# LBM-EPFL/MaD

Measured on NVIDIA B200. Metric: voxels/sec scale-space+detect+describe(+match), higher is better.
Workload: dtype f32 grids, f64 line accumulation, u8 x u8 -> s32 matching

## Files before the change

### include/mad_b200.h

```cpp
#ifndef MAD_B200_H
#define MAD_B200_H

#include <stddef.h>
#include <stdint.h>

#ifdef __cplusplus
extern "C" {
#endif

#define MAD_OK 0
#define MAD_ERR_ARG (-1)
#define MAD_ERR_CUDA (-2)
#define MAD_ERR_CAPACITY (-3)
#define MAD_ERR_NODEVICE (-4)

#define MAD_MAX_ORI 36
#define MAD_DSC_LEN 1024
#define MAD_DSC_REFUSED (1 << 30)

typedef struct MadKeypoint {
    int32_t vox[3];
    int32_t oct;
    float off[3];
    float val;
    int32_t peak[3];
    int32_t accepted;
} MadKeypoint;

typedef struct MadOriented {
    int32_t kp;
    int16_t main_bin;
    int16_t sec_bin;
} MadOriented;

typedef struct MadZoneTable {
    int32_t n_zones;
    int32_t n_belts;
    const double* bounds;
    const int32_t* belt_first;
    const double* belt_phi;
    const void* fast;
} MadZoneTable;

#define MAD_ZONE_FAST_BYTES 2048
int mad_zone_fast_build(const MadZoneTable* zones_host, void* fast_out, void* stream);

const char* mad_last_error_string(void);
int mad_version(void);
int mad_device_info(int* sm_count, int* cc_major, int* cc_minor);

int mad_publish_small(const void* src_dev, void* dst_host_mapped, int bytes, void* stream);

int mad_copy_to_host(const void* src_dev, void* dst_host_mapped, long long bytes, int n_ctas, void* stream);

long long mad_launch_count(void);
int mad_profile_enable(int on);
int mad_profile_count(void);
int mad_profile_get(int i, const char** name, float* ms);
int mad_profile_reset(void);

int mad_grid_max(const float* grid, long long n, float* out_max_ord, void* stream);
float mad_grid_max_decode(unsigned int ord);
int mad_threshold_normalise(float* grid, long long n, float isovalue, float vmax, int divide, void* stream);
int mad_grid_bbox(const float* grid, int nx, int ny, int nz, int* bbox6, void* stream);
int mad_crop_pad3d(const float* in, int nx, int ny, int nz, int x0, int y0, int z0, int cx, int cy, int cz,
                   int pad, float* out, void* stream);

int mad_pad3d(const float* in, int nx, int ny, int nz, int pad, float* out, void* stream);

size_t mad_upsample_workspace_bytes(int bx, int by, int bz);
int mad_upsample_presmooth(const float* base, int bx, int by, int bz,
                           const double* gauss_w_host, int radius,
                           float* up, void* workspace, size_t workspace_bytes, void* stream);

size_t mad_log_gauss_workspace_bytes(int nx, int ny, int nz);
int mad_log_gauss(const float* grid, int nx, int ny, int nz,
                  const double* w0_host, const double* w2_host, int radius, float scale,
                  float* log_out, float* gauss_out, void* workspace, size_t workspace_bytes,
                  int exact_f64, void* stream);

int mad_gradient(const float* gauss, int nx, int ny, int nz, float* grad4, void* stream);
size_t mad_gradient_tiles(int nx, int ny, int nz);
int mad_gradient_mark(const MadKeypoint* kp, int n_kp, const int* dims_oct_host, int reach_oct0, int reach_oct1,
                      uint8_t* flags_oct0, uint8_t* flags_oct1, void* stream);
int mad_gradient_masked(const float* gauss, int nx, int ny, int nz, float* grad4, uint8_t* flags, void* stream);

int mad_detect(const float* log_grid, int nx, int ny, int nz, int oct, int border,
               float threshold, MadKeypoint* cand, int cap, int* count, void* stream);

size_t mad_sort_keypoints_workspace_bytes(int n);
int mad_sort_keypoints(const MadKeypoint* cand, int n, const int* dims_oct_host,
                       MadKeypoint* out, int* out_count,
                       void* workspace, size_t workspace_bytes, void* stream);

int mad_orient(const float* grad4_oct0, const float* grad4_oct1, const int* dims_oct_host,
               const MadKeypoint* kp, int n_kp, int r, const MadZoneTable* zones112_host,
               const double* r1_table, int lim_main, int lim_sec,
               int32_t* n_ori, int32_t* slots, void* stream);

size_t mad_compact_oriented_workspace_bytes(int n_kp);
int mad_compact_oriented(const int32_t* n_ori, const int32_t* slots, int n_kp,
                         MadOriented* oriented, int cap, int* out_count,
                         void* workspace, size_t workspace_bytes, void* stream);

int mad_describe(const float* grad4_oct0, const float* grad4_oct1, const int* dims_oct_host,
                 const MadKeypoint* kp, const MadOriented* oriented, int n_oriented, int r,
                 const MadZoneTable* zones16_host, const double* rf_table, const double* rf_inv_table,
                 int rf_zones, int16_t* dsc, void* stream);

typedef struct MadDscSet {
    const int16_t* dsc;
    const void* half;
    const int32_t* norm2;
    const uint8_t* u8;
    const float* rnorm;
    int32_t rows;
    int32_t rows_padded;
    int32_t max_entry;
    int32_t max_norm2;
} MadDscSet;

int mad_dsc_prepare(const int16_t* dsc, int rows, int rows_padded, int32_t* norm2, float* rnorm,
                    uint8_t* u8, int32_t* max_entry, int32_t* max_norm2, void* stream);
int mad_dsc_norms(const int16_t* dsc, int rows, int32_t* norm2, void* stream);
int mad_dsc_to_half(const int16_t* dsc, int rows, int rows_padded, void* half_out, void* stream);

int mad_match_segments(int M, int N, int impl);
int mad_match_count(const MadDscSet* hi, const MadDscSet* lo, double cc, int n_seg, int32_t* seg_count, int impl,
                    void* stream);
int mad_match_fill(const MadDscSet* hi, const MadDscSet* lo, double cc, int n_seg, const int64_t* seg_offset,
                   int32_t* pair_hi, int32_t* pair_lo, double* pair_score, int impl, void* stream);
size_t mad_exclusive_scan_workspace_bytes(int n);
int mad_exclusive_scan_i32_to_i64(const int32_t* in, int n, int64_t* out, int64_t* total,
                                  void* workspace, size_t workspace_bytes, void* stream);

int mad_match_pairs(const MadDscSet* hi, const MadDscSet* lo, double cc, uint64_t* cand_key, int32_t* cand_dot,
                    uint64_t cap, uint64_t* count, void* stream);
size_t mad_match_pairs_finish_workspace_bytes(long long n);
int mad_match_pairs_finish(const uint64_t* cand_key, const int32_t* cand_dot, long long n, int hi_rows, int lo_rows,
                           const int32_t* hi_n2, const int32_t* lo_n2, int32_t* pair_hi, int32_t* pair_lo,
                           double* pair_score, void* workspace, size_t workspace_bytes, void* stream);
int mad_match_pairs_finish_dot(const uint64_t* cand_key, const int32_t* cand_dot, long long n, int hi_rows, int lo_rows,
                               int32_t* pair_hi, int32_t* pair_lo, int32_t* pair_dot, void* workspace, size_t workspace_bytes,
                               void* stream);

size_t mad_match_topk_workspace_bytes(int M, int N, int k, int impl);
int mad_match_topk(const MadDscSet* hi, const MadDscSet* lo, int k, int lo_index_base,
                   int32_t* topk_idx, double* topk_score, void* workspace, size_t workspace_bytes,
                   int impl, void* stream);
#define MAD_TOPK_INCOMPLETE (-2)
int mad_topk_merge(const int32_t* idx_in, const double* score_in, int G, int M, int k,
                   int32_t* idx_out, double* score_out, void* stream);

int mad_mark_used(const int32_t* idx, long long n, uint8_t* used, void* stream);
int mad_repeatability(const int32_t* pair_hi, const int32_t* pair_lo, const double* pair_score, long long n_pairs,
                      const double* hi_subv, const double* lo_subv, const int32_t* hi_meta, const int32_t* lo_meta,
                      const double* rf_table, const double* rf_inv_table, int rf_zones,
                      const double* hi_cloud, int n_hi_cloud, const double* lo_sorted, const int32_t* cell_start,
                      const uint32_t* near_bits, const double* grid_org_host, const int* grid_dims_host,
                      double dist, double* results, void* stream);
int mad_repeat_counts(const int32_t* pair_hi, const int32_t* pair_lo, long long p0, long long p1,
                      const double* hi_subv, const double* lo_subv, const int32_t* hi_meta, const int32_t* lo_meta,
                      const double* rf_table, const double* rf_inv_table, int rf_zones,
                      const double* hi_cloud, int n_hi_cloud, const double* lo_sorted, const int32_t* cell_start,
                      const uint32_t* near_bits, const double* grid_org_host, const int* grid_dims_host,
                      double dist, int32_t* counts, void* stream);
int mad_repeat_rows(const int32_t* pair_hi, const int32_t* pair_lo, const double* pair_score, long long n_pairs,
                    const double* hi_subv, const double* lo_subv, const int32_t* hi_meta, const int32_t* lo_meta,
                    const double* rf_table, const double* rf_inv_table, int rf_zones, const int32_t* counts,
                    int n_hi_cloud, double* results, void* stream);

size_t mad_anchor_cloud_workspace_bytes(int n_rows);
int mad_anchor_cloud(const double* subv, const uint8_t* used, int n_rows, double cell, double* cloud, double* grid_org,
                     long long* info, void* workspace, size_t workspace_bytes, void* stream);
size_t mad_cloud_grid_workspace_bytes(int n);
int mad_cloud_grid(const double* cloud, int n, const double* grid_org, const long long* grid_dims_host, double cell,
                   double* sorted, int32_t* cell_start, uint32_t* near_bits, void* workspace, size_t workspace_bytes,
                   void* stream);

int mad_density_splat(const double* xyz, const double* mass, int n_atoms, const double* min_host, double voxelsp,
                      int margin, int px, int py, int pz, double* grid, void* stream);
int mad_normalise_f64(double* grid, long long n, void* scratch8, void* stream);
int mad_conv_full_f64(const double* in, long long outer, int n, long long inner, const double* w_dev, int radius,
                      void* out, int out_is_f32, void* stream);

size_t mad_box_scores_workspace_bytes(int ex, int ey, int ez);
int mad_box_scores(const float* g1, int nx1, int ny1, int nz1, const float* g2, int nx2, int ny2, int nz2,
                   const int* box_host, float isovalue, double* out8, void* workspace, size_t workspace_bytes,
                   void* stream);
int mad_grid_count_gt(const float* grid, long long n, float thr, unsigned long long* out, void* stream);
int mad_mask_with(float* g1, int nx1, int ny1, int nz1, const float* g2, int nx2, int ny2, int nz2,
                  const int* shift_host, const int* lo_host, const int* hi_host, void* stream);
int mad_refine_rigid(const float* grad4, int nx, int ny, int nz, const double* px, const double* py, const double* pz,
                     double voxsp, const double* init, const double* center, const double* max_dist, int n_problems,
                     int n_atoms, int n_steps, double max_step, double min_step, double* coords_out, double* meta_out,
                     void* stream);

#ifdef __cplusplus
}
#endif
#endif
```

### mad_b200/_lib.py

```python
import ctypes as C
import os

import numpy as np

HERE = os.path.dirname(os.path.abspath(__file__))
LIB_PATH = os.path.join(HERE, "libmad_b200.so")


class MadError(RuntimeError):
    pass


if not os.path.exists(LIB_PATH):
    raise ImportError(
        "mad_b200: %s is missing -- build the CUDA library first (python -m mad_b200.build). "
        "There is no CPU fallback." % LIB_PATH)

lib = C.CDLL(LIB_PATH)

KEYPOINT_DTYPE = np.dtype([("vox", "<i4", 3), ("oct", "<i4"), ("off", "<f4", 3), ("val", "<f4"),
                           ("peak", "<i4", 3), ("accepted", "<i4")])
ORIENTED_DTYPE = np.dtype([("kp", "<i4"), ("main", "<i2"), ("sec", "<i2")])
assert KEYPOINT_DTYPE.itemsize == 48 and ORIENTED_DTYPE.itemsize == 8
MAX_ORI = 36
DSC_LEN = 1024
DSC_REFUSED = 1 << 30
TOPK_INCOMPLETE = -2
TOPK_MAX = 32
ZONE_FAST_BYTES = 2048


class MadZoneTable(C.Structure):
    _fields_ = [("n_zones", C.c_int32), ("n_belts", C.c_int32), ("bounds", C.c_void_p),
                ("belt_first", C.c_void_p), ("belt_phi", C.c_void_p), ("fast", C.c_void_p)]


class MadDscSet(C.Structure):
    _fields_ = [("dsc", C.c_void_p), ("half", C.c_void_p), ("norm2", C.c_void_p), ("u8", C.c_void_p),
                ("rnorm", C.c_void_p), ("rows", C.c_int32), ("rows_padded", C.c_int32), ("max_entry", C.c_int32),
                ("max_norm2", C.c_int32)]


_P = C.c_void_p
_I = C.c_int
_SZ = C.c_size_t

SIGNATURES = {
    "mad_last_error_string": (C.c_char_p, []),
    "mad_version": (_I, []),
    "mad_device_info": (_I, [C.POINTER(_I), C.POINTER(_I), C.POINTER(_I)]),
    "mad_launch_count": (C.c_longlong, []),
    "mad_profile_enable": (_I, [_I]),
    "mad_profile_count": (_I, []),
    "mad_profile_get": (_I, [_I, C.POINTER(C.c_char_p), C.POINTER(C.c_float)]),
    "mad_profile_reset": (_I, []),
    "mad_publish_small": (_I, [_P, _P, _I, _P]),
    "mad_copy_to_host": (_I, [_P, _P, C.c_longlong, _I, _P]),
    "mad_zone_fast_build": (_I, [C.POINTER(MadZoneTable), _P, _P]),
    "mad_grid_max": (_I, [_P, C.c_longlong, _P, _P]),
    "mad_grid_max_decode": (C.c_float, [C.c_uint]),
    "mad_threshold_normalise": (_I, [_P, C.c_longlong, C.c_float, C.c_float, _I, _P]),
    "mad_grid_bbox": (_I, [_P, _I, _I, _I, _P, _P]),
    "mad_crop_pad3d": (_I, [_P, _I, _I, _I, _I, _I, _I, _I, _I, _I, _I, _P, _P]),
    "mad_pad3d": (_I, [_P, _I, _I, _I, _I, _P, _P]),
    "mad_upsample_workspace_bytes": (_SZ, [_I, _I, _I]),
    "mad_upsample_presmooth": (_I, [_P, _I, _I, _I, _P, _I, _P, _P, _SZ, _P]),
    "mad_log_gauss_workspace_bytes": (_SZ, [_I, _I, _I]),
    "mad_log_gauss": (_I, [_P, _I, _I, _I, _P, _P, _I, C.c_float, _P, _P, _P, _SZ, _I, _P]),
    "mad_gradient": (_I, [_P, _I, _I, _I, _P, _P]),
    "mad_gradient_tiles": (_SZ, [_I, _I, _I]),
    "mad_gradient_mark": (_I, [_P, _I, _P, _I, _I, _P, _P, _P]),
    "mad_gradient_masked": (_I, [_P, _I, _I, _I, _P, _P, _P]),
    "mad_detect": (_I, [_P, _I, _I, _I, _I, _I, C.c_float, _P, _I, _P, _P]),
    "mad_sort_keypoints_workspace_bytes": (_SZ, [_I]),
    "mad_sort_keypoints": (_I, [_P, _I, _P, _P, _P, _P, _SZ, _P]),
    "mad_orient": (_I, [_P, _P, _P, _P, _I, _I, C.POINTER(MadZoneTable), _P, _I, _I, _P, _P, _P]),
    "mad_compact_oriented_workspace_bytes": (_SZ, [_I]),
    "mad_compact_oriented": (_I, [_P, _P, _I, _P, _I, _P, _P, _SZ, _P]),
    "mad_describe": (_I, [_P, _P, _P, _P, _P, _I, _I, C.POINTER(MadZoneTable), _P, _P, _I, _P, _P]),
    "mad_dsc_prepare": (_I, [_P, _I, _I, _P, _P, _P, _P, _P, _P]),
    "mad_match_pairs": (_I, [C.POINTER(MadDscSet), C.POINTER(MadDscSet), C.c_double, _P, _P, C.c_uint64, _P, _P]),
    "mad_match_pairs_finish_workspace_bytes": (_SZ, [C.c_longlong]),
    "mad_match_pairs_finish": (_I, [_P, _P, C.c_longlong, _I, _I, _P, _P, _P, _P, _P, _P, _SZ, _P]),
    "mad_match_pairs_finish_dot": (_I, [_P, _P, C.c_longlong, _I, _I, _P, _P, _P, _P, _SZ, _P]),
    "mad_dsc_norms": (_I, [_P, _I, _P, _P]),
    "mad_dsc_to_half": (_I, [_P, _I, _I, _P, _P]),
    "mad_match_segments": (_I, [_I, _I, _I]),
    "mad_match_count": (_I, [C.POINTER(MadDscSet), C.POINTER(MadDscSet), C.c_double, _I, _P, _I, _P]),
    "mad_match_fill": (_I, [C.POINTER(MadDscSet), C.POINTER(MadDscSet), C.c_double, _I, _P, _P, _P, _P, _I, _P]),
    "mad_exclusive_scan_workspace_bytes": (_SZ, [_I]),
    "mad_exclusive_scan_i32_to_i64": (_I, [_P, _I, _P, _P, _P, _SZ, _P]),
    "mad_match_topk_workspace_bytes": (_SZ, [_I, _I, _I, _I]),
    "mad_match_topk": (_I, [C.POINTER(MadDscSet), C.POINTER(MadDscSet), _I, _I, _P, _P, _P, _SZ, _I, _P]),
    "mad_topk_merge": (_I, [_P, _P, _I, _I, _I, _P, _P, _P]),
    "mad_density_splat": (_I, [_P, _P, _I, _P, C.c_double, _I, _I, _I, _I, _P, _P]),
    "mad_normalise_f64": (_I, [_P, C.c_longlong, _P, _P]),
    "mad_conv_full_f64": (_I, [_P, C.c_longlong, _I, C.c_longlong, _P, _I, _P, _I, _P]),
    "mad_mark_used": (_I, [_P, C.c_longlong, _P, _P]),
    "mad_repeatability": (_I, [_P, _P, _P, C.c_longlong, _P, _P, _P, _P, _P, _P, _I, _P, _I, _P, _P, _P, _P, _P,
                               C.c_double, _P, _P]),
    "mad_repeat_counts": (_I, [_P, _P, C.c_longlong, C.c_longlong, _P, _P, _P, _P, _P, _P, _I, _P, _I, _P, _P, _P, _P, _P,
                               C.c_double, _P, _P]),
    "mad_repeat_rows": (_I, [_P, _P, _P, C.c_longlong, _P, _P, _P, _P, _P, _P, _I, _P, _I, _P, _P]),
    "mad_anchor_cloud_workspace_bytes": (_SZ, [_I]),
    "mad_anchor_cloud": (_I, [_P, _P, _I, C.c_double, _P, _P, _P, _P, _SZ, _P]),
    "mad_cloud_grid_workspace_bytes": (_SZ, [_I]),
    "mad_cloud_grid": (_I, [_P, _I, _P, _P, C.c_double, _P, _P, _P, _P, _SZ, _P]),
    "mad_box_scores_workspace_bytes": (_SZ, [_I, _I, _I]),
    "mad_box_scores": (_I, [_P, _I, _I, _I, _P, _I, _I, _I, _P, C.c_float, _P, _P, _SZ, _P]),
    "mad_grid_count_gt": (_I, [_P, C.c_longlong, C.c_float, _P, _P]),
    "mad_mask_with": (_I, [_P, _I, _I, _I, _P, _I, _I, _I, _P, _P, _P, _P]),
    "mad_refine_rigid": (_I, [_P, _I, _I, _I, _P, _P, _P, C.c_double, _P, _P, _P, _I, _I, _I, C.c_double, C.c_double,
                              _P, _P, _P]),
}

for _name, (_res, _args) in SIGNATURES.items():
    _f = getattr(lib, _name)
    _f.restype = _res
    _f.argtypes = _args


def last_error():
    s = lib.mad_last_error_string()
    return s.decode() if s else ""


def check(rc, what):
    if rc != 0:
        raise MadError("%s failed with status %d: %s" % (what, rc, last_error()))


def call(name, *args):
    check(getattr(lib, name)(*args), name)
```

### mad_b200/csrc/describe.cu

```cuda
#include "common.cuh"
#include "eqsp_zones.cuh"

namespace {

struct OctDims { int n[2][3]; };

__device__ __forceinline__ int nearest_idx(double p) { return __double2loint(__dadd_ru(p - 0.5, 6755399441055744.0)); }

__device__ __noinline__ int zone_exact_dsc(ZoneTab T, const double* __restrict__ Rm, float gx, float gy, float gz) {
    const double vx0 = gx, vy0 = gy, vz0 = gz;
    const double vx = (vx0 * Rm[0] + vy0 * Rm[1]) + vz0 * Rm[2];
    const double vy = (vx0 * Rm[3] + vy0 * Rm[4]) + vz0 * Rm[5];
    const double vz = (vx0 * Rm[6] + vy0 * Rm[7]) + vz0 * Rm[8];
    double th = atan2(vy, vx);
    if (th < 0.0) th += MAD_TWO_PI;
    const double sth = th + MAD_TWO_PI;
    const double ph = acos(fmin(1.0, fmax(-1.0, vz)));
    int z[2];
    const int nzn = zones_of(T, th, sth, ph, z);
    if (nzn == 1) return z[0];
    if (nzn >= 2) return max(z[0], z[1]);
    return 0;
}

template <int NB, int SIDE, int THREADS>
__global__ void __launch_bounds__(THREADS, 768 / THREADS)
describe_kernel(const float4* __restrict__ grad0, const float4* __restrict__ grad1, OctDims dims,
                const MadKeypoint* __restrict__ kp, const MadOriented* __restrict__ oriented, int r,
                ZoneTab T, const double* __restrict__ rf_table, const double* __restrict__ rf_inv_table,
                int rf_zones, int16_t* __restrict__ dsc) {
    __shared__ int cnt[MAD_DSC_LEN];
    __shared__ ZoneFast F;
    __shared__ double xt[32][3];
    const int tid = threadIdx.x;
    if (SIDE) r = SIDE / 2;
    const MadOriented of = oriented[blockIdx.x];
    const MadKeypoint K = kp[of.kp];
    const int o = K.oct ? 1 : 0;
    const float4* __restrict__ grad = o ? grad1 : grad0;
    const int nx = dims.n[o][0], ny = dims.n[o][1], nz = dims.n[o][2];
    const long long tab = ((long long)of.main_bin * rf_zones + of.sec_bin) * 9;
    double Ri[9];
    float Rmf[9];
#pragma unroll
    for (int q = 0; q < 9; ++q) { Ri[q] = rf_inv_table[tab + q]; Rmf[q] = (float)rf_table[tab + q]; }
    const int side = SIDE ? SIDE : 2 * r;
    const int c1 = r / 2, c2 = r, c3 = (3 * r) / 2;
    const double cx = K.vox[0], cy = K.vox[1], cz = K.vox[2];
    const double u0 = o ? (-(double)r + 0.5) : (double)(-2 * r + 1);
    const double du = o ? 1.0 : 2.0;

    for (int q = tid; q < MAD_DSC_LEN; q += blockDim.x) cnt[q] = 0;
    zone_fast_init(&F, T);
    if (tid < side) {
        const double lx = u0 + du * tid;
        xt[tid][0] = lx * Ri[0]; xt[tid][1] = lx * Ri[3]; xt[tid][2] = lx * Ri[6];
    }

    int bad = 0;
    if (tid < 8) {
        const double lx = u0 + du * ((tid & 1) ? side - 1 : 0);
        const double ly = u0 + du * ((tid & 2) ? side - 1 : 0);
        const double lz = u0 + du * ((tid & 4) ? side - 1 : 0);
        const double px = ((lx * Ri[0] + ly * Ri[1]) + lz * Ri[2]) + cx;
        const double py = ((lx * Ri[3] + ly * Ri[4]) + lz * Ri[5]) + cy;
        const double pz = ((lx * Ri[6] + ly * Ri[7]) + lz * Ri[8]) + cz;
        bad = (px < 0.0 || px > (double)(nx - 1) || py < 0.0 || py > (double)(ny - 1) || pz < 0.0 || pz > (double)(nz - 1));
    }
    const int s_bad = __syncthreads_or(bad);
    float vz_hi[NB];
    zone_fast_hi<NB>(F, vz_hi);
    int16_t* out = dsc + (long long)blockIdx.x * MAD_DSC_LEN;
    if (s_bad) {
        for (int q = tid; q < MAD_DSC_LEN; q += blockDim.x) out[q] = 0;
        return;
    }

    constexpr int GB = 4;
    const int plane = side * side;
    for (int c = tid; c < plane; c += blockDim.x) {
        const int k = c % side, j = c / side;
        const double ly = u0 + du * j, lz = u0 + du * k;
        const double ay0 = ly * Ri[1], ay1 = ly * Ri[4], ay2 = ly * Ri[7];
        const double az0 = lz * Ri[2], az1 = lz * Ri[5], az2 = lz * Ri[8];
        const int by = (j >= c1) + (j >= c2) + (j >= c3);
        const int bz = (k >= c1) + (k >= c2) + (k >= c3);
        const int bin_jk = (16 * by + bz) * T.n_zones;
#pragma unroll 1
        for (int i0 = 0; i0 < (SIDE ? SIDE : side); i0 += GB) {
            float4 gv[GB];
#pragma unroll
            for (int u = 0; u < GB; ++u) {
                const int i = SIDE ? i0 + u : min(i0 + u, side - 1);
                const double px = ((xt[i][0] + ay0) + az0) + cx;
                const double py = ((xt[i][1] + ay1) + az1) + cy;
                const double pz = ((xt[i][2] + ay2) + az2) + cz;
                const int ix = nearest_idx(px), iy = nearest_idx(py), iz = nearest_idx(pz);
                gv[u] = __ldg(grad + (unsigned)((ix * ny + iy) * nz + iz));
            }
            float vx[GB], vy[GB], vz[GB];
            bool valid[GB];
#pragma unroll
            for (int u = 0; u < GB; ++u) {
                const float4 g = gv[u];
                const float m2 = __fadd_rn(__fadd_rn(__fmul_rn(g.x, g.x), __fmul_rn(g.y, g.y)), __fmul_rn(g.z, g.z));
                valid[u] = (SIDE || i0 + u < side) && !(m2 < MAD_M2_LT);
                const float rinv = mad_rsqrt_approx(fmaxf(m2, 1e-30f));
                vx[u] = ((g.x * Rmf[0] + g.y * Rmf[1]) + g.z * Rmf[2]) * rinv;
                vy[u] = ((g.x * Rmf[3] + g.y * Rmf[4]) + g.z * Rmf[5]) * rinv;
                vz[u] = ((g.x * Rmf[6] + g.y * Rmf[7]) + g.z * Rmf[8]) * rinv;
            }
            int zone[GB];
#pragma unroll
            for (int u = 0; u < GB; ++u) zone[u] = zone_fast<NB>(F, vz_hi, vx[u], vy[u], vz[u]);
#pragma unroll
            for (int u = 0; u < GB; ++u) {
                if (valid[u]) {
                    if (zone[u] < 0) {
                        const float4 g = gv[u];
                        const float m = __fsqrt_rn(__fadd_rn(__fadd_rn(__fmul_rn(g.x, g.x), __fmul_rn(g.y, g.y)), __fmul_rn(g.z, g.z)));
                        zone[u] = zone_exact_dsc(T, rf_table + tab, __fdiv_rn(g.x, m), __fdiv_rn(g.y, m), __fdiv_rn(g.z, m));
                    }
                    const int i = i0 + u;
                    const int bx = (i >= c1) + (i >= c2) + (i >= c3);
                    atomicAdd(&cnt[bin_jk + 4 * bx * T.n_zones + zone[u]], 1);
                }
            }
        }
    }
    __syncthreads();
    for (int q = tid; q < MAD_DSC_LEN; q += blockDim.x) out[q] = (int16_t)cnt[q];
}

}

extern "C" int mad_describe(const float* grad4_oct0, const float* grad4_oct1, const int* dims_oct_host,
                            const MadKeypoint* kp, const MadOriented* oriented, int n_oriented, int r,
                            const MadZoneTable* zones_host, const double* rf_table, const double* rf_inv_table,
                            int rf_zones, int16_t* dsc, void* stream) {
    MAD_CHECK_ARG(dims_oct_host && zones_host && n_oriented >= 0);
    if (n_oriented == 0) return MAD_OK;
    MAD_CHECK_ARG(grad4_oct0 && grad4_oct1 && kp && oriented && rf_table && rf_inv_table && dsc);
    MAD_CHECK_ARG(zones_host->n_zones * 64 == MAD_DSC_LEN);
    MAD_CHECK_ARG(r >= 2 && r <= 16 && rf_zones > 0);
    OctDims d;
    for (int o = 0; o < 2; ++o) for (int a = 0; a < 3; ++a) d.n[o][a] = dims_oct_host[3 * o + a];
    ZoneTab T;
    T.bounds = zones_host->bounds; T.belt_first = zones_host->belt_first; T.belt_phi = zones_host->belt_phi;
    T.n_zones = zones_host->n_zones; T.n_belts = zones_host->n_belts; T.fast = zones_host->fast;
    MAD_CHECK_ARG(T.n_belts >= 1 && T.n_belts <= MAD_BELT_MAX && T.n_zones <= MAD_ZONE_MAX);
    MAD_PROF("describe_kernel", stream);
    for (int o = 0; o < 2; ++o)
        MAD_CHECK_ARG((long long)d.n[o][0] * d.n[o][1] * d.n[o][2] < (1LL << 31));
    auto launch = [&](auto kernel, int threads) {
        kernel<<<n_oriented, threads, 0, (cudaStream_t)stream>>>(
            reinterpret_cast<const float4*>(grad4_oct0), reinterpret_cast<const float4*>(grad4_oct1), d, kp, oriented, r,
            T, rf_table, rf_inv_table, rf_zones, dsc);
    };
    if (T.n_belts <= 4 && r == 8) launch(describe_kernel<4, 16, 128>, 128);
    else if (T.n_belts <= 4) launch(describe_kernel<4, 0, 256>, 256);
    else launch(describe_kernel<MAD_BELT_MAX, 0, 256>, 256);
    MAD_LAUNCH_OK();
    return MAD_OK;
}
```

### mad_b200/csrc/orient.cu

```cuda
#include <cub/cub.cuh>

#include "common.cuh"
#include "eqsp_zones.cuh"

namespace {

struct OctDims { int n[2][3]; };

__device__ __forceinline__ int norm50(int h, int hmax) {
    return (int)((double)h / (double)hmax * 50.0);
}

__device__ __forceinline__ void normalise_exact(float& gx, float& gy, float& gz) {
    const float m = __fsqrt_rn(__fadd_rn(__fadd_rn(__fmul_rn(gx, gx), __fmul_rn(gy, gy)), __fmul_rn(gz, gz)));
    if (m > 1e-5f) {
        gx = __fdiv_rn(gx, m);
        gy = __fdiv_rn(gy, m);
        gz = __fdiv_rn(gz, m);
    }
}
__device__ __noinline__ void vote_exact_f32(ZoneTab T, float gx, float gy, float gz, int* hist) {
    normalise_exact(gx, gy, gz);
    float th = (float)atan2((double)gy, (double)gx);
    if (th < 0.f) th = __fadd_rn(th, 6.2831855f);
    const float sth = __fadd_rn(th, 6.2831855f);
    const float zc = fminf(1.f, fmaxf(-1.f, gz));
    const float ph = (float)acos((double)zc);
    int z[2];
    const int nzn = zones_of(T, (double)th, (double)sth, (double)ph, z);
    if (nzn > 0) atomicAdd(&hist[z[0]], 1);
    if (nzn > 1) atomicAdd(&hist[z[1]], 1);
}
__device__ __noinline__ void vote_exact_f64(ZoneTab T, const double* __restrict__ R, float gx, float gy, float gz, int* hist) {
    normalise_exact(gx, gy, gz);
    const double px = gx, py = gy, pz = gz;
    const double vx = fma(pz, R[2], fma(py, R[1], px * R[0]));
    const double vy = fma(pz, R[5], fma(py, R[4], px * R[3]));
    const double vz = fma(pz, R[8], fma(py, R[7], px * R[6]));
    double th = atan2(vy, vx);
    if (th < 0.0) th += MAD_TWO_PI;
    const double sth = th + MAD_TWO_PI;
    const double ph = acos(fmin(1.0, fmax(-1.0, vz)));
    int z[2];
    const int nzn = zones_of(T, th, sth, ph, z);
    if (nzn > 0) atomicAdd(&hist[z[0]], 1);
    if (nzn > 1) atomicAdd(&hist[z[1]], 1);
}

__device__ __forceinline__ int select_zones(bool flag, int zone, int* out, int* warp_cnt) {
    const int lane = threadIdx.x & 31, warp = threadIdx.x >> 5;
    const unsigned m = __ballot_sync(0xFFFFFFFFu, flag);
    if (lane == 0) warp_cnt[warp] = __popc(m);
    __syncthreads();
    int base = 0, total = 0;
    const int nw = blockDim.x >> 5;
    for (int w = 0; w < nw; ++w) { const int c = warp_cnt[w]; if (w < warp) base += c; total += c; }
    if (flag) {
        const int p = base + __popc(m & ((1u << lane) - 1u));
        if (p < 8) out[p] = zone;
    }
    __syncthreads();
    return total;
}

template <int NB>
__global__ void __launch_bounds__(128)
orient_kernel(const float4* __restrict__ grad0, const float4* __restrict__ grad1, OctDims dims,
              const MadKeypoint* __restrict__ kp, int r, const char4* __restrict__ mask_off, int n_mask,
              ZoneTab T, const double* __restrict__ r1_table, int lim_main, int lim_sec,
              int32_t* __restrict__ n_ori, int32_t* __restrict__ slots) {
    extern __shared__ float4 pv[];
    __shared__ int hist[128];
    __shared__ int hn0[128];
    __shared__ int cur[128];
    __shared__ int s_main[8], s_sec[8], s_wcnt[8];
    __shared__ int s_hmax, s_count;
    __shared__ ZoneFast F;

    const int tid = threadIdx.x;
    const int ki = blockIdx.x;
    const MadKeypoint K = kp[ki];
    const int o = K.oct ? 1 : 0;
    const float4* __restrict__ grad = o ? grad1 : grad0;
    const int nx = dims.n[o][0], ny = dims.n[o][1], nz = dims.n[o][2];
    const int s = o ? 1 : 2;
    const int cx = K.vox[0], cy = K.vox[1], cz = K.vox[2];
    if (cx - s * r < 0 || cy - s * r < 0 || cz - s * r < 0 ||
        cx + s * r + 1 > nx - 1 || cy + s * r + 1 > ny - 1 || cz + s * r + 1 > nz - 1) {
        if (tid == 0) n_ori[ki] = 0;
        return;
    }
    if (tid < 128) { hist[tid] = 0; }
    if (tid == 0) { s_hmax = 0; s_count = 0; }
    zone_fast_init(&F, T);
    __syncthreads();
    float vz_hi[NB];
    zone_fast_hi<NB>(F, vz_hi);

    constexpr int GB = 4;
    for (int i0 = tid; i0 < n_mask; i0 += GB * blockDim.x) {
        float4 gv[GB];
#pragma unroll
        for (int u = 0; u < GB; ++u) {
            const int i = i0 + u * blockDim.x;
            gv[u] = make_float4(0.f, 0.f, 0.f, 0.f);
            if (i < n_mask) {
                const char4 d = mask_off[i];
                const long long idx = ((long long)(cx + s * d.x) * ny + (cy + s * d.y)) * nz + (cz + s * d.z);
                gv[u] = __ldg(grad + idx);
            }
        }
        int zf[GB];
#pragma unroll
        for (int u = 0; u < GB; ++u) {
            float4 g = gv[u];
            const float m2 = __fadd_rn(__fadd_rn(__fmul_rn(g.x, g.x), __fmul_rn(g.y, g.y)), __fmul_rn(g.z, g.z));
            const float rinv = mad_rsqrt_approx(fmaxf(m2, 1e-30f));
            g.w = (m2 < MAD_M2_LT) ? 0.f : ((m2 >= MAD_M2_GT) ? rinv : -1.f);
            gv[u] = g;
            zf[u] = (g.w > 0.f) ? zone_fast<NB>(F, vz_hi, g.x * rinv, g.y * rinv, g.z * rinv) : -1;
        }
#pragma unroll
        for (int u = 0; u < GB; ++u) {
            const int i = i0 + u * blockDim.x;
            if (i < n_mask) {
                pv[i] = gv[u];
                if (gv[u].w != 0.f) {
                    if (zf[u] >= 0) atomicAdd(&hist[zf[u]], 1);
                    else vote_exact_f32(T, gv[u].x, gv[u].y, gv[u].z, hist);
                }
            }
        }
    }
    __syncthreads();
    if (tid < T.n_zones) atomicMax(&s_hmax, hist[tid]);
    __syncthreads();
    const int hmax0 = s_hmax;
    if (hmax0 == 0) {
        if (tid == 0) n_ori[ki] = 0;
        return;
    }
    if (tid < T.n_zones) hn0[tid] = norm50(hist[tid], hmax0);
    __syncthreads();
    const int nmain = select_zones(tid < T.n_zones && hn0[tid] > 40, tid, s_main, s_wcnt);
    if (nmain > lim_main) {
        if (tid == 0) n_ori[ki] = 0;
        return;
    }

    for (int mi = 0; mi < nmain; ++mi) {
        const int a = s_main[mi];
        bool have = true;
        if (a != 0) {
            if (tid < 128) hist[tid] = 0;
            if (tid == 0) s_hmax = 0;
            __syncthreads();
            const double* R = r1_table + 9 * a;
            float rf[9];
#pragma unroll
            for (int q = 0; q < 9; ++q) rf[q] = (float)R[q];
            for (int i0 = tid; i0 < n_mask; i0 += GB * blockDim.x) {
                float4 gq[GB];
                int zq[GB];
#pragma unroll
                for (int u = 0; u < GB; ++u) {
                    const int i = min(i0 + u * (int)blockDim.x, n_mask - 1);
                    const float4 g = pv[i];
                    gq[u] = g;
                    const float vx = fmaf(g.z, rf[2], fmaf(g.y, rf[1], g.x * rf[0])) * g.w;
                    const float vy = fmaf(g.z, rf[5], fmaf(g.y, rf[4], g.x * rf[3])) * g.w;
                    const float vz = fmaf(g.z, rf[8], fmaf(g.y, rf[7], g.x * rf[6])) * g.w;
                    zq[u] = (g.w > 0.f) ? zone_fast<NB>(F, vz_hi, vx, vy, vz) : -1;
                }
#pragma unroll
                for (int u = 0; u < GB; ++u) {
                    if (i0 + u * (int)blockDim.x < n_mask && gq[u].w != 0.f) {
                        if (zq[u] >= 0) atomicAdd(&hist[zq[u]], 1);
                        else vote_exact_f64(T, R, gq[u].x, gq[u].y, gq[u].z, hist);
                    }
                }
            }
            __syncthreads();
            if (tid < T.n_zones) atomicMax(&s_hmax, hist[tid]);
            __syncthreads();
            const int hm = s_hmax;
            if (hm == 0) have = false;
            else if (tid < T.n_zones) cur[tid] = norm50(hist[tid], hm);
        } else {
            if (tid < T.n_zones) cur[tid] = hn0[tid];
        }
        __syncthreads();
        if (tid == 0) s_hmax = 0;
        __syncthreads();
        const bool inner = tid >= 1 && tid < T.n_zones - 1;
        if (have && inner) atomicMax(&s_hmax, cur[tid]);
        __syncthreads();
        const int qmax = s_hmax;
        const int ns = select_zones(have && inner && qmax > 0 && norm50(cur[tid], max(qmax, 1)) > 40, tid, s_sec, s_wcnt);
        if (tid == 0 && have && qmax > 0 && ns <= lim_sec) {
            int c = s_count;
            for (int q = 0; q < ns && c < MAD_MAX_ORI; ++q) slots[(long long)ki * MAD_MAX_ORI + c++] = a | (s_sec[q] << 16);
            s_count = c;
        }
        __syncthreads();
    }
    if (tid == 0) n_ori[ki] = s_count;
}

__global__ void compact_oriented_kernel(const int32_t* __restrict__ n_ori, const int32_t* __restrict__ slots,
                                        const int* __restrict__ pos, int n_kp, MadOriented* __restrict__ out,
                                        int cap, int* __restrict__ out_count) {
    const int i = blockIdx.x * blockDim.x + threadIdx.x;
    if (i >= n_kp) return;
    const int n = n_ori[i], p = pos[i];
    for (int q = 0; q < n; ++q) {
        if (p + q < cap) {
            const int v = slots[(long long)i * MAD_MAX_ORI + q];
            MadOriented of;
            of.kp = i;
            of.main_bin = (int16_t)(v & 0xFFFF);
            of.sec_bin = (int16_t)(v >> 16);
            out[p + q] = of;
        }
    }
    if (i == n_kp - 1) *out_count = p + n;
}

}

static char4* g_mask_dev[32] = {nullptr};
static int g_mask_count[32] = {0};

static int ensure_mask(int r, const char4** dev, int* count) {
    if (r < 1 || r >= 32) return MAD_ERR_ARG;
    if (!g_mask_dev[r]) {
        const double lim = r * 1.05;
        const int side = 2 * r + 1;
        char4* host = (char4*)malloc(sizeof(char4) * side * side * side);
        int n = 0;
        for (int dx = -r; dx <= r; ++dx)
            for (int dy = -r; dy <= r; ++dy)
                for (int dz = -r; dz <= r; ++dz)
                    if (sqrt((double)(dx * dx + dy * dy + dz * dz)) <= lim) {
                        host[n].x = (signed char)dx; host[n].y = (signed char)dy; host[n].z = (signed char)dz; host[n].w = 0;
                        ++n;
                    }
        char4* d = nullptr;
        if (cudaMalloc(&d, sizeof(char4) * n) != cudaSuccess) { free(host); return MAD_ERR_CUDA; }
        if (cudaMemcpy(d, host, sizeof(char4) * n, cudaMemcpyHostToDevice) != cudaSuccess) { free(host); return MAD_ERR_CUDA; }
        free(host);
        g_mask_dev[r] = d;
        g_mask_count[r] = n;
    }
    *dev = g_mask_dev[r];
    *count = g_mask_count[r];
    return MAD_OK;
}

extern "C" int mad_orient(const float* grad4_oct0, const float* grad4_oct1, const int* dims_oct_host,
                          const MadKeypoint* kp, int n_kp, int r, const MadZoneTable* zones_host,
                          const double* r1_table, int lim_main, int lim_sec, int32_t* n_ori, int32_t* slots,
                          void* stream) {
    MAD_CHECK_ARG(dims_oct_host && zones_host && r1_table && n_kp >= 0);
    if (n_kp == 0) return MAD_OK;
    MAD_CHECK_ARG(grad4_oct0 && grad4_oct1 && kp && n_ori && slots);
    MAD_CHECK_ARG(zones_host->n_zones >= 3 && zones_host->n_zones <= 128 && zones_host->n_belts < 32);
    MAD_CHECK_ARG(lim_main >= 0 && lim_main <= 6 && lim_sec >= 0 && lim_sec <= 6);
    const char4* mask = nullptr;
    int n_mask = 0;
    int rc = ensure_mask(r, &mask, &n_mask);
    if (rc != MAD_OK) { mad_set_error("mad_orient: cannot build the spherical mask for r=%d", r); return rc; }
    OctDims d;
    for (int o = 0; o < 2; ++o) for (int a = 0; a < 3; ++a) d.n[o][a] = dims_oct_host[3 * o + a];
    ZoneTab T;
    T.bounds = zones_host->bounds; T.belt_first = zones_host->belt_first; T.belt_phi = zones_host->belt_phi;
    T.n_zones = zones_host->n_zones; T.n_belts = zones_host->n_belts; T.fast = zones_host->fast;
    const size_t smem = (size_t)n_mask * sizeof(float4);
    if (smem > 200 * 1024) { mad_set_error("mad_orient: patch radius %d too large", r); return MAD_ERR_ARG; }
    MAD_CHECK_ARG(T.n_belts >= 1 && T.n_belts <= MAD_BELT_MAX && T.n_zones <= MAD_ZONE_MAX);
    auto launch = [&](auto kernel) -> int {
        MAD_CUDA(cudaFuncSetAttribute(kernel, cudaFuncAttributeMaxDynamicSharedMemorySize, (int)std::max<size_t>(smem, 48 * 1024)));
        MAD_PROF("orient_kernel", stream);
        kernel<<<n_kp, 128, smem, (cudaStream_t)stream>>>(

            reinterpret_cast<const float4*>(grad4_oct0), reinterpret_cast<const float4*>(grad4_oct1), d, kp, r, mask,
            n_mask, T, r1_table, lim_main, lim_sec, n_ori, slots);
        return MAD_OK;
    };
    int lrc;
    if (T.n_belts <= 4) lrc = launch(orient_kernel<4>);
    else if (T.n_belts <= 12) lrc = launch(orient_kernel<12>);
    else lrc = launch(orient_kernel<MAD_BELT_MAX>);
    if (lrc != MAD_OK) return lrc;
    MAD_LAUNCH_OK();
    return MAD_OK;
}

__global__ void zone_fast_build_kernel(ZoneTab T, ZoneFast* out) {
    __shared__ ZoneFast F;
    zone_fast_init(&F, T);
    __syncthreads();
    const uint32_t* src = reinterpret_cast<const uint32_t*>(&F);
    uint32_t* dst = reinterpret_cast<uint32_t*>(out);
    for (int i = threadIdx.x; i < (int)(sizeof(ZoneFast) / 4); i += blockDim.x) dst[i] = src[i];
}

extern "C" int mad_zone_fast_build(const MadZoneTable* zones_host, void* fast_out, void* stream) {
    MAD_CHECK_ARG(zones_host && fast_out && zones_host->bounds && zones_host->belt_first && zones_host->belt_phi);
    MAD_CHECK_ARG(zones_host->n_zones >= 1 && zones_host->n_zones <= MAD_ZONE_MAX);
    MAD_CHECK_ARG(zones_host->n_belts >= 1 && zones_host->n_belts <= MAD_BELT_MAX);
    MAD_CHECK_ARG((reinterpret_cast<uintptr_t>(fast_out) & 15) == 0);
    ZoneTab T;
    T.bounds = zones_host->bounds; T.belt_first = zones_host->belt_first; T.belt_phi = zones_host->belt_phi;
    T.n_zones = zones_host->n_zones; T.n_belts = zones_host->n_belts; T.fast = nullptr;
    MAD_PROF("zone_fast_build_kernel", stream);
    zone_fast_build_kernel<<<1, 128, 0, (cudaStream_t)stream>>>(T, reinterpret_cast<ZoneFast*>(fast_out));
    MAD_LAUNCH_OK();
    return MAD_OK;
}

extern "C" size_t mad_compact_oriented_workspace_bytes(int n_kp) {
    size_t b = 0;
    cub::DeviceScan::ExclusiveSum(nullptr, b, (const int*)nullptr, (int*)nullptr, n_kp > 0 ? n_kp : 1);
    return mad_align_up((size_t)(n_kp > 0 ? n_kp : 1) * sizeof(int), 256) + mad_align_up(b, 256);
}

extern "C" int mad_compact_oriented(const int32_t* n_ori, const int32_t* slots, int n_kp, MadOriented* oriented,
                                    int cap, int* out_count, void* workspace, size_t workspace_bytes, void* stream) {
    MAD_CHECK_ARG(out_count && n_kp >= 0);
    cudaStream_t st = (cudaStream_t)stream;
    if (n_kp == 0) {
        MAD_CUDA(cudaMemsetAsync(out_count, 0, sizeof(int), st));
        return MAD_OK;
    }
    MAD_CHECK_ARG(n_ori && slots && oriented && workspace && cap >= 0);
    MAD_CHECK_ARG(workspace_bytes >= mad_compact_oriented_workspace_bytes(n_kp));
    int* pos = reinterpret_cast<int*>(workspace);
    char* cub_ws = reinterpret_cast<char*>(workspace) + mad_align_up((size_t)n_kp * sizeof(int), 256);
    size_t cub_bytes = workspace_bytes - mad_align_up((size_t)n_kp * sizeof(int), 256);
    {
        MAD_PROF("cub_exclusive_sum", st);
        MAD_CUDA(cub::DeviceScan::ExclusiveSum(cub_ws, cub_bytes, n_ori, pos, n_kp, st));
    }
    MAD_PROF("compact_oriented_kernel", st);
    compact_oriented_kernel<<<(int)mad_ceil_div(n_kp, 256), 256, 0, st>>>(n_ori, slots, pos, n_kp, oriented, cap, out_count);
    MAD_LAUNCH_OK();
    return MAD_OK;
}
```

### mad_b200/pipeline.py

```python
import ctypes as C
import math
import os

import numpy as np
import torch

from . import _lib
from . import tables
from ._lib import call, KEYPOINT_DTYPE, ORIENTED_DTYPE, MAX_ORI, DSC_LEN

def launch_count():
    return int(_lib.lib.mad_launch_count())


def profile_enable(on=True):
    call("mad_profile_reset")
    call("mad_profile_enable", 1 if on else 0)


def profile_records():
    out = []
    name = C.c_char_p()
    ms = C.c_float()
    for i in range(_lib.lib.mad_profile_count()):
        call("mad_profile_get", i, C.byref(name), C.byref(ms))
        out.append((name.value.decode(), float(ms.value)))
    call("mad_profile_reset")
    return out


def _require_cuda():
    if not torch.cuda.is_available():
        raise _lib.MadError("mad_b200 needs a CUDA device (sm_100a); there is no CPU fallback")


def _stream():
    return C.c_void_p(torch.cuda.current_stream().cuda_stream)


def _ptr(t):
    return C.c_void_p(t.data_ptr()) if t is not None else C.c_void_p(0)


class _Readback(object):
    _slots = {}

    @classmethod
    def read(cls, *tensors):
        dev = tensors[0].device
        key = (dev.index, torch.cuda.current_stream().cuda_stream)
        slot = cls._slots.get(key)
        if slot is None:
            slot = cls._slots[key] = torch.zeros(512, dtype=torch.int64).pin_memory()
        st = _stream()
        off, views = 0, []
        for t in tensors:
            t = t.contiguous().view(-1)
            nbytes = t.numel() * t.element_size()
            assert nbytes % 4 == 0 and off + nbytes <= slot.numel() * 8
            call("mad_publish_small", _ptr(t), C.c_void_p(slot.data_ptr() + off), nbytes, st)
            views.append((off, t.dtype, t.numel()))
            off += (nbytes + 7) // 8 * 8
        torch.cuda.current_stream().synchronize()
        raw = slot.numpy()
        out = []
        for o, dt, n in views:
            a = raw.view(np.uint8)[o:o + n * (8 if dt == torch.int64 else 4)].view(np.int64 if dt == torch.int64 else np.int32)
            out.extend(int(v) for v in a)
        return out


def _dptr(a):
    return a.ctypes.data_as(C.c_void_p)


class _DeviceTables(object):

    def __init__(self, device, ori_zones=112, dsc_zones=16):
        self.device = device
        self.keep = []
        self.z_ori = self._zone_struct(tables.zone_tables(ori_zones))
        self.z_dsc = self._zone_struct(tables.zone_tables(dsc_zones))
        ot = tables.orientation_tables(ori_zones)
        self.ori_zones = ori_zones
        self.r1 = torch.from_numpy(np.ascontiguousarray(ot.r1.reshape(-1, 9))).to(device)
        self.rf = torch.from_numpy(np.ascontiguousarray(ot.rf.reshape(-1, 9))).to(device)
        self.rf_inv = torch.from_numpy(np.ascontiguousarray(ot.rf_inv.reshape(-1, 9))).to(device)

    def _zone_struct(self, zt):
        b = torch.from_numpy(np.ascontiguousarray(zt.bounds)).to(self.device)
        f = torch.from_numpy(np.ascontiguousarray(zt.belt_first)).to(self.device)
        p = torch.from_numpy(np.ascontiguousarray(zt.belt_phi)).to(self.device)
        self.keep += [b, f, p]
        s = _lib.MadZoneTable()
        s.n_zones, s.n_belts = zt.size, zt.n_belts
        s.bounds, s.belt_first, s.belt_phi = b.data_ptr(), f.data_ptr(), p.data_ptr()
        s.fast = None
        fast = torch.zeros(_lib.ZONE_FAST_BYTES, dtype=torch.uint8, device=self.device)
        with torch.cuda.device(self.device):
            call("mad_zone_fast_build", C.byref(s), _ptr(fast), _stream())
            torch.cuda.current_stream().synchronize()
        self.keep.append(fast)
        s.fast = fast.data_ptr()
        return s


_TABLE_CACHE = {}


def device_tables(device):
    key = (str(device),)
    if key not in _TABLE_CACHE:
        _TABLE_CACHE[key] = _DeviceTables(device)
    return _TABLE_CACHE[key]


class Space(object):

    def __init__(self):
        self.grids = []
        self.logs = []
        self.gauss = []
        self.grad4 = []
        self.grad_flags = []
        self.dims = []
        self.n_oct = 2
        self.n_input_voxels = 0
        self._gauss = []
        self._grad_done = {}

    @property
    def dims_host(self):
        return np.array([d for o in self.dims for d in o], dtype=np.int32)


def gradient_reach(radius):
    up = max(2 * radius, int(math.ceil((2 * radius - 1) * math.sqrt(3.0))) + 1)
    base = max(radius, int(math.ceil((radius - 0.5) * math.sqrt(3.0))) + 1)
    return up, base


def ensure_gradient(space, kp, radius=8):
    if all(f is None for f in space.grad_flags[:space.n_oct]) or len(kp) == 0:
        return
    key = (id(kp), int(radius))
    if key in space._grad_done:
        return
    st = _stream()
    up, base = gradient_reach(int(radius))
    f0, f1 = space.grad_flags
    if f0 is None or f1 is None:
        raise _lib.MadError("ensure_gradient: octaves must share the gradient mode")
    call("mad_gradient_mark", _ptr(kp.table), len(kp), _dptr(space.dims_host), up, base, _ptr(f0), _ptr(f1), st)
    for o, (gx, gy, gz) in enumerate(space.dims[:space.n_oct]):
        call("mad_gradient_masked", _ptr(space._gauss[o]), gx, gy, gz, _ptr(space.grad4[o]), _ptr(space.grad_flags[o]), st)
    space._grad_done[key] = kp


def full_gradient(space):
    st = _stream()
    for o, (gx, gy, gz) in enumerate(space.dims[:space.n_oct]):
        fl = space.grad_flags[o]
        if fl is None:
            continue
        fl[fl == 0] = 1
        call("mad_gradient_masked", _ptr(space._gauss[o]), gx, gy, gz, _ptr(space.grad4[o]), _ptr(fl), st)
        space.grad_flags[o] = None
    space.grad_flags = [None] * len(space.grad_flags)
    return space.grad4


def build_space(grid, map_padding=9, sig_init=2, sig_presmooth=1, exact_f64=True, keep_gauss=True, full_gradient=True,
                oct_mode="both"):
    _require_cuda()
    if isinstance(grid, np.ndarray):
        grid = torch.from_numpy(np.ascontiguousarray(grid, dtype=np.float32)).cuda()
    grid = grid.contiguous().float()
    dev = grid.device
    st = _stream()
    nx, ny, nz = grid.shape
    sp = Space()
    sp.n_input_voxels = nx * ny * nz
    if map_padding:
        bx, by, bz = nx + 2 * map_padding, ny + 2 * map_padding, nz + 2 * map_padding
        base = torch.empty((bx, by, bz), dtype=torch.float32, device=dev)
        call("mad_pad3d", _ptr(grid), nx, ny, nz, int(map_padding), _ptr(base), st)
    else:
        bx, by, bz = nx, ny, nz
        base = grid
    if oct_mode not in ("both", "up", "base"):
        raise _lib.MadError("build_space: oct_mode %r" % (oct_mode,))
    ux, uy, uz = 2 * bx - 1, 2 * by - 1, 2 * bz - 1
    if oct_mode != "base":
        up = torch.empty((ux, uy, uz), dtype=torch.float32, device=dev)
        ws_bytes = _lib.lib.mad_upsample_workspace_bytes(bx, by, bz)
        ws = torch.empty(ws_bytes, dtype=torch.uint8, device=dev)
        if sig_presmooth:
            rad = tables.gaussian_radius(sig_presmooth)
            gw = np.ascontiguousarray(tables.gaussian_weights(sig_presmooth, 0, rad))
            call("mad_upsample_presmooth", _ptr(base), bx, by, bz, _dptr(gw), rad, _ptr(up), _ptr(ws), ws_bytes, st)
        else:
            call("mad_upsample_presmooth", _ptr(base), bx, by, bz, C.c_void_p(0), 0, _ptr(up), _ptr(ws), ws_bytes, st)
        del ws
    if oct_mode == "both":
        sp.grids = [up, base]
        sp.dims = [(ux, uy, uz), (bx, by, bz)]
    else:
        sp.n_oct = 1
        sp.grids = [up] if oct_mode == "up" else [base]
        sp.dims = [(ux, uy, uz) if oct_mode == "up" else (bx, by, bz)]
    rad = tables.gaussian_radius(sig_init)
    w0 = np.ascontiguousarray(tables.gaussian_weights(sig_init, 0, rad))
    w2 = np.ascontiguousarray(tables.gaussian_weights(sig_init, 2, rad))
    scale = float(np.float32(sig_init ** 2))
    for g, (gx, gy, gz) in zip(sp.grids, sp.dims):
        ws_bytes = _lib.lib.mad_log_gauss_workspace_bytes(gx, gy, gz)
        ws = torch.empty(ws_bytes, dtype=torch.uint8, device=dev)
        lg = torch.empty((gx, gy, gz), dtype=torch.float32, device=dev)
        gs = torch.empty((gx, gy, gz), dtype=torch.float32, device=dev)
        call("mad_log_gauss", _ptr(g), gx, gy, gz, _dptr(w0), _dptr(w2), rad, C.c_float(scale), _ptr(lg), _ptr(gs),
             _ptr(ws), ws_bytes, 1 if exact_f64 else 0, st)
        del ws
        gr = torch.empty((gx, gy, gz, 4), dtype=torch.float32, device=dev)
        if full_gradient:
            call("mad_gradient", _ptr(gs), gx, gy, gz, _ptr(gr), st)
            sp.grad_flags.append(None)
        else:
            sp.grad_flags.append(torch.zeros(_lib.lib.mad_gradient_tiles(gx, gy, gz), dtype=torch.uint8, device=dev))
        sp._gauss.append(gs)
        sp.logs.append(lg)
        sp.gauss.append(gs if keep_gauss else None)
        sp.grad4.append(gr)
    if full_gradient and not keep_gauss:
        sp._gauss = []
    if sp.n_oct == 1:
        sp.dims.append((1, 1, 1))
        sp.grad4.append(torch.zeros((1, 1, 1, 4), dtype=torch.float32, device=dev))
        sp.grad_flags.append(None if full_gradient else torch.zeros(1, dtype=torch.uint8, device=dev))
    return sp


class Keypoints(object):

    def __init__(self, table, count):
        self.table = table
        self.count = int(count)
        self._host = None

    def host(self):
        if self._host is None:
            self._host = self.table[:self.count].cpu().numpy().view(KEYPOINT_DTYPE).reshape(-1)
        return self._host

    def __len__(self):
        return self.count


def keypoints_from_host(arr, device):
    arr = np.ascontiguousarray(arr, dtype=KEYPOINT_DTYPE)
    t = torch.from_numpy(arr.view(np.int32).reshape(-1, 12).copy()).to(device)
    k = Keypoints(t, len(arr))
    k._host = arr
    return k


def detect(space, border=12, threshold=5e-2, cap=None):
    _require_cuda()
    dev = space.logs[0].device
    st = _stream()
    if cap is None:
        cap = 1 << 16
    while True:
        cand = torch.empty((cap, 12), dtype=torch.int32, device=dev)
        counter = torch.zeros(1, dtype=torch.int32, device=dev)
        for o, (lg, (gx, gy, gz)) in enumerate(zip(space.logs, space.dims)):
            call("mad_detect", _ptr(lg), gx, gy, gz, o, int(border), C.c_float(threshold), _ptr(cand), cap,
                 _ptr(counter), st)
        n = _Readback.read(counter)[0]
        if n <= cap:
            break
        cap = int(n * 1.25) + 16
    out = torch.empty((max(n, 1), 12), dtype=torch.int32, device=dev)
    out_count = torch.zeros(1, dtype=torch.int32, device=dev)
    ws_bytes = _lib.lib.mad_sort_keypoints_workspace_bytes(n)
    ws = torch.empty(max(ws_bytes, 1), dtype=torch.uint8, device=dev)
    dims = space.dims_host
    call("mad_sort_keypoints", _ptr(cand), n, _dptr(dims), _ptr(out), _ptr(out_count), _ptr(ws), ws_bytes, st)
    return Keypoints(out, _Readback.read(out_count)[0])


class Oriented(object):
    def __init__(self, table, count):
        self.table = table
        self.count = int(count)
        self._host = None

    def host(self):
        if self._host is None:
            self._host = self.table[:self.count].cpu().numpy().view(ORIENTED_DTYPE).reshape(-1)
        return self._host

    def __len__(self):
        return self.count


def oriented_from_host(arr, device):
    arr = np.ascontiguousarray(arr, dtype=ORIENTED_DTYPE)
    t = torch.from_numpy(arr.view(np.int32).reshape(-1, 2).copy()).to(device)
    o = Oriented(t, len(arr))
    o._host = arr
    return o


def orient(space, kp, radius=8, lim_main=6, lim_sec=6):
    _require_cuda()
    dev = space.grad4[0].device
    st = _stream()
    tb = device_tables(dev)
    n = len(kp)
    if n == 0:
        return Oriented(torch.empty((1, 2), dtype=torch.int32, device=dev), 0)
    ensure_gradient(space, kp, radius)
    n_ori = torch.empty(n, dtype=torch.int32, device=dev)
    slots = torch.empty((n, MAX_ORI), dtype=torch.int32, device=dev)
    dims = space.dims_host
    call("mad_orient", _ptr(space.grad4[0]), _ptr(space.grad4[1]), _dptr(dims), _ptr(kp.table), n, int(radius),
         C.byref(tb.z_ori), _ptr(tb.r1), int(lim_main), int(lim_sec), _ptr(n_ori), _ptr(slots), st)
    cap = n * MAX_ORI
    out = torch.empty((cap, 2), dtype=torch.int32, device=dev)
    out_count = torch.zeros(1, dtype=torch.int32, device=dev)
    ws_bytes = _lib.lib.mad_compact_oriented_workspace_bytes(n)
    ws = torch.empty(ws_bytes, dtype=torch.uint8, device=dev)
    call("mad_compact_oriented", _ptr(n_ori), _ptr(slots), n, _ptr(out), cap, _ptr(out_count), _ptr(ws), ws_bytes, st)
    return Oriented(out, _Readback.read(out_count)[0])


def describe(space, kp, ori, radius=8):
    _require_cuda()
    dev = space.grad4[0].device
    st = _stream()
    tb = device_tables(dev)
    d = len(ori)
    dsc = torch.empty((d, DSC_LEN), dtype=torch.int16, device=dev)
    if d == 0:
        return dsc
    ensure_gradient(space, kp, radius)
    dims = space.dims_host
    call("mad_describe", _ptr(space.grad4[0]), _ptr(space.grad4[1]), _dptr(dims), _ptr(kp.table), _ptr(ori.table), d,
         int(radius), C.byref(tb.z_dsc), _ptr(tb.rf), _ptr(tb.rf_inv), tb.ori_zones, _ptr(dsc), st)
    return dsc


def describe_struct(grid, patch_size=16, map_padding=9, sig_init=2, sig_presmooth=1, exact_f64=True,
                    keep_gauss=False, full_gradient=None):
    r = (patch_size - patch_size % 2) // 2
    if full_gradient is None:
        full_gradient = bool(keep_gauss)
    sp = build_space(grid, map_padding, sig_init, sig_presmooth, exact_f64=exact_f64, keep_gauss=keep_gauss,
                     full_gradient=full_gradient)
    kp = detect(sp)
    ori = orient(sp, kp, r)
    dsc = describe(sp, kp, ori, r)
    return sp, kp, ori, dsc


class DescriptorSet(object):

    def __init__(self, dsc, need_half=False):
        _require_cuda()
        if isinstance(dsc, np.ndarray):
            dsc = torch.from_numpy(np.ascontiguousarray(dsc, dtype=np.int16)).cuda()
        self.dsc = dsc.contiguous()
        assert self.dsc.dtype == torch.int16 and self.dsc.dim() == 2 and self.dsc.shape[1] == DSC_LEN
        dev = self.dsc.device
        st = _stream()
        self.rows = self.dsc.shape[0]
        self.rows_padded = max((self.rows + 255) // 256 * 256, 256)
        self.norm2 = torch.empty(max(self.rows, 1), dtype=torch.int32, device=dev)
        self.rnorm = torch.empty(self.rows_padded, dtype=torch.float32, device=dev)
        self.u8 = torch.empty((self.rows_padded, DSC_LEN), dtype=torch.uint8, device=dev)
        mx = torch.zeros(2, dtype=torch.int32, device=dev)
        call("mad_dsc_prepare", _ptr(self.dsc), self.rows, self.rows_padded, _ptr(self.norm2), _ptr(self.rnorm),
             _ptr(self.u8), _ptr(mx), _ptr(mx[1:]), st)
        self._max_dev = mx
        self._max_entry = None
        self._max_norm2 = None
        self.half = None
        s = _lib.MadDscSet()
        s.dsc = self.dsc.data_ptr()
        s.half = 0
        s.norm2 = self.norm2.data_ptr()
        s.u8 = self.u8.data_ptr()
        s.rnorm = self.rnorm.data_ptr()
        s.rows, s.rows_padded = self.rows, self.rows_padded
        s.max_entry = -1
        s.max_norm2 = -1
        self.c = s
        if need_half:
            self.ensure_half()

    @property
    def max_entry(self):
        if self._max_entry is None:
            self._set_maxima(*self._max_dev.tolist())
        return self._max_entry

    def _set_maxima(self, max_entry, max_norm2):
        self._max_entry, self._max_norm2 = int(max_entry), int(max_norm2)
        self.c.max_entry, self.c.max_norm2 = self._max_entry, self._max_norm2

    def ensure_half(self):
        if self.half is None:
            self.half = torch.empty((self.rows_padded, DSC_LEN), dtype=torch.float16, device=self.dsc.device)
            call("mad_dsc_to_half", _ptr(self.dsc), self.rows, self.rows_padded, _ptr(self.half), _stream())
            self.c.half = self.half.data_ptr()
        return self


def _as_set(x):
    return x if isinstance(x, DescriptorSet) else DescriptorSet(x)


def _check_descriptors(hi, lo):
    if max(hi._max_entry, lo._max_entry) >= _lib.DSC_REFUSED:
        raise _lib.MadError("mad_match: not a descriptor set (a negative entry, or a squared norm >= 2^31)")


def _exact_impl(hi, lo):
    _check_descriptors(hi, lo)
    if max(hi._max_entry, lo._max_entry) <= 255:
        return 0
    if max(hi._max_entry, lo._max_entry) <= 2048 and hi._max_norm2 * lo._max_norm2 <= 1 << 48:
        return 2
    return 1


def _pick_impl(hi, lo, impl):
    verify = False
    if impl is None:
        if hi._max_entry is None or lo._max_entry is None:
            return 0, True
        impl = _exact_impl(hi, lo)
    return _pick_impl_explicit(hi, lo, impl), verify


def _pick_impl_explicit(hi, lo, impl):
    hi.max_entry, lo.max_entry
    if impl == 2:
        hi.ensure_half()
        lo.ensure_half()
    return impl


_PAIR_CAP = {}


def scores_from_dots(pair_hi, pair_lo, pair_dot, hi_norm2, lo_norm2):
    p = np.asarray(hi_norm2, dtype=np.float64)[np.asarray(pair_hi)] * np.asarray(lo_norm2, dtype=np.float64)[np.asarray(pair_lo)]
    out = np.zeros(len(p), dtype=np.float64)
    nz = p > 0.0
    out[nz] = np.asarray(pair_dot, dtype=np.float64)[nz] / np.sqrt(p[nz])
    return out


def pair_hi_from_counts(counts):
    counts = np.asarray(counts)
    return np.repeat(np.arange(len(counts), dtype=np.int32), counts)


def match_threshold(hi, lo, cc=0.6, impl=None, want="score"):
    hi, lo = _as_set(hi), _as_set(lo)
    dev = hi.dsc.device
    st = _stream()
    m = hi.rows
    if m == 0 or lo.rows == 0:
        e = torch.empty(0, dtype=torch.int32, device=dev)
        return e, e.clone(), torch.empty(0, dtype=torch.float64, device=dev)
    impl, verify = _pick_impl(hi, lo, impl)
    if impl == 0:
        return _match_threshold_onepass(hi, lo, cc, dev, st, verify, want)
    if want != "score":
        raise _lib.MadError("match_threshold: want='dot' is a format of the uint8 kernel (impl 0)")
    n_seg = int(_lib.lib.mad_match_segments(m, lo.rows, impl))
    seg_count = torch.empty(m * n_seg, dtype=torch.int32, device=dev)
    call("mad_match_count", C.byref(hi.c), C.byref(lo.c), C.c_double(cc), n_seg, _ptr(seg_count), impl, st)
    seg_off = torch.empty(m * n_seg, dtype=torch.int64, device=dev)
    total = torch.zeros(1, dtype=torch.int64, device=dev)
    ws_bytes = _lib.lib.mad_exclusive_scan_workspace_bytes(m * n_seg)
    ws = torch.empty(ws_bytes, dtype=torch.uint8, device=dev)
    call("mad_exclusive_scan_i32_to_i64", _ptr(seg_count), m * n_seg, _ptr(seg_off), _ptr(total), _ptr(ws), ws_bytes, st)
    p = int(total.item())
    pair_hi = torch.empty(max(p, 1), dtype=torch.int32, device=dev)
    pair_lo = torch.empty(max(p, 1), dtype=torch.int32, device=dev)
    score = torch.empty(max(p, 1), dtype=torch.float64, device=dev)
    call("mad_match_fill", C.byref(hi.c), C.byref(lo.c), C.c_double(cc), n_seg, _ptr(seg_off), _ptr(pair_hi), _ptr(pair_lo),
         _ptr(score), impl, st)
    return pair_hi[:p], pair_lo[:p], score[:p]


def _read_counts(count, hi, lo):
    vals = _Readback.read(count, hi._max_dev, lo._max_dev)
    hi._set_maxima(vals[1], vals[2])
    lo._set_maxima(vals[3], vals[4])
    return int(vals[0])


def _match_threshold_onepass(hi, lo, cc, dev, st, verify=False, want="score"):
    key = (hi.rows, lo.rows)
    cap = _PAIR_CAP.get(key, max(1 << 20, 16 * (hi.rows + lo.rows)))
    while True:
        cand_key = torch.empty(cap, dtype=torch.int64, device=dev)
        cand_dot = torch.empty(cap, dtype=torch.int32, device=dev)
        count = torch.empty(1, dtype=torch.int64, device=dev)
        call("mad_match_pairs", C.byref(hi.c), C.byref(lo.c), C.c_double(cc), _ptr(cand_key), _ptr(cand_dot),
             C.c_uint64(cap), _ptr(count), st)
        p = _read_counts(count, hi, lo)
        if p >= (1 << 62):
            raise _lib.MadError("mad_match_pairs: the kernel's internal hand-off timed out (pair list incomplete)")
        if verify and _exact_impl(hi, lo) != 0:
            if want != "score":
                raise _lib.MadError("match_threshold: entries above 255 need the fp16 or SIMT kernel, which have no want='dot' form")
            return match_threshold(hi, lo, cc)
        if p <= cap:
            break
        cap = p + p // 8 + 1024
    _PAIR_CAP[key] = max(cap, p + p // 4)
    pair_hi = torch.empty(max(p, 1), dtype=torch.int32, device=dev)
    pair_lo = torch.empty(max(p, 1), dtype=torch.int32, device=dev)
    score = torch.empty(max(p, 1), dtype=torch.float64 if want == "score" else torch.int32, device=dev)
    if p:
        ws_bytes = _lib.lib.mad_match_pairs_finish_workspace_bytes(p)
        ws = torch.empty(ws_bytes, dtype=torch.uint8, device=dev)
        if want == "score":
            call("mad_match_pairs_finish", _ptr(cand_key), _ptr(cand_dot), p, hi.rows, lo.rows, _ptr(hi.norm2), _ptr(lo.norm2),
                 _ptr(pair_hi), _ptr(pair_lo), _ptr(score), _ptr(ws), ws_bytes, st)
        else:
            call("mad_match_pairs_finish_dot", _ptr(cand_key), _ptr(cand_dot), p, hi.rows, lo.rows, _ptr(pair_hi), _ptr(pair_lo),
                 _ptr(score), _ptr(ws), ws_bytes, st)
    return pair_hi[:p], pair_lo[:p], score[:p]


HOST_COPY_CTAS = int(os.environ.get("MAD_HOST_COPY_CTAS", "8"))


class HostStage(object):

    def __init__(self):
        self.bufs = {}
        self.copy_stream = None
        self.keep = []

    def fetch(self, name, t, overlap=False):
        n = t.numel() * t.element_size()
        buf = self.bufs.get(name)
        if buf is None or buf.numel() < n:
            if buf is not None:
                self.keep.append(buf)
            buf = torch.empty(max(n * 5 // 4, 256), dtype=torch.uint8).pin_memory()
            self.bufs[name] = buf
        view = buf[:n].view(t.dtype).view(t.shape)
        if not n:
            return view
        if overlap:
            if self.copy_stream is None:
                self.copy_stream = torch.cuda.Stream()
            self.copy_stream.wait_stream(torch.cuda.current_stream())
            t = t.contiguous()
            if t.data_ptr() % 16 == 0:
                call("mad_copy_to_host", _ptr(t), C.c_void_p(buf.data_ptr()), n, HOST_COPY_CTAS, C.c_void_p(self.copy_stream.cuda_stream))
            else:
                with torch.cuda.stream(self.copy_stream):
                    view.copy_(t, non_blocking=True)
            t.record_stream(self.copy_stream)
            self.keep.append(t)
        else:
            view.copy_(t, non_blocking=True)
        return view

    def sync(self):
        torch.cuda.current_stream().synchronize()
        if self.copy_stream is not None:
            self.copy_stream.synchronize()
        self.keep = []
        self.marks = []

    def mark(self):
        evs = [torch.cuda.Event()]
        evs[0].record(torch.cuda.current_stream())
        if self.copy_stream is not None:
            evs.append(torch.cuda.Event())
            evs[1].record(self.copy_stream)
        self.marks = evs

    def wait(self):
        for ev in getattr(self, "marks", []):
            ev.synchronize()
        self.marks = []
        self.keep = []


class MapStream(object):

    def __init__(self, hi=None, cc=0.6, exact_f64=True, match_impl=None, patch_size=16, depth=2, download=True, compact=False):
        _require_cuda()
        self.compact = bool(compact)
        self.download = download
        self.hi = _as_set(hi) if hi is not None else None
        self.cc, self.exact, self.impl, self.patch = cc, exact_f64, match_impl, patch_size
        self.up_stream = torch.cuda.Stream()
        self.stages = [HostStage() for _ in range(max(2, depth))]
        self.n = 0
        self.gbuf = [None] * max(2, depth)
        self.gfree = [None] * max(2, depth)
        self.n_up = 0

    def upload(self, grid):
        if isinstance(grid, np.ndarray):
            grid = torch.from_numpy(np.ascontiguousarray(grid, dtype=np.float32))
        if self.n_up - self.n >= len(self.gbuf):
            raise _lib.MadError("MapStream.upload: %d uploads are waiting for submit(); the %d upload buffers are all in use"
                                % (self.n_up - self.n, len(self.gbuf)))
        k = self.n_up % len(self.gbuf)
        self.n_up += 1
        dev = torch.device("cuda", torch.cuda.current_device())
        if self.gbuf[k] is None or self.gbuf[k].shape != grid.shape:
            self.gbuf[k] = torch.empty(tuple(grid.shape), dtype=torch.float32, device=dev)
        if self.gfree[k] is not None:
            self.up_stream.wait_event(self.gfree[k])
        with torch.cuda.stream(self.up_stream):
            self.gbuf[k].copy_(grid, non_blocking=True)
            ev = torch.cuda.Event()
            ev.record(self.up_stream)
        return self.gbuf[k], ev, k

    def submit(self, uploaded):
        g, ev, k = uploaded
        cur = torch.cuda.current_stream()
        cur.wait_event(ev)
        stage = self.stages[self.n % len(self.stages)]
        self.n += 1
        stage.wait()
        sp, kp, ori, dsc = describe_struct(g, patch_size=self.patch, exact_f64=self.exact)
        if k is not None:
            self.gfree[k] = torch.cuda.Event()
            self.gfree[k].record(cur)
        get = (lambda name, t: stage.fetch(name, t, overlap=True)) if self.download else (lambda name, t: t)
        out = {"kp": get("kp", kp.table[:len(kp)]), "ori": get("ori", ori.table[:len(ori)])}
        lo = DescriptorSet(dsc) if (self.hi is not None or self.compact) else None
        if self.compact:
            out.update(dsc_u8=get("dsc8", lo.u8[:lo.rows]), lo_norm2=get("n2", lo.norm2[:lo.rows]))
        else:
            out["dsc"] = get("dsc", dsc)
        if self.hi is not None:
            if self.compact:
                ph, pl, dot = match_threshold(self.hi, lo, self.cc, impl=self.impl, want="dot")
                cnt = torch.zeros(self.hi.rows, dtype=torch.int32, device=ph.device)
                if ph.numel():
                    cnt.scatter_add_(0, ph.long(), torch.ones_like(ph))
                out.update(pair_hi_counts=get("pc", cnt), pair_lo=get("pl", pl), pair_dot=get("pd", dot))
            else:
                ph, pl, sc = match_threshold(self.hi, lo, self.cc, impl=self.impl)
                out.update(pair_hi=get("ph", ph), pair_lo=get("pl", pl), score=get("sc", sc))
        stage.mark()
        return stage, out

    def result(self, ticket):
        stage, out = ticket
        stage.wait()
        return out


class MapBatch(object):

    def __init__(self, streams=4, patch_size=16, exact_f64=True, compact=False):
        _require_cuda()
        from concurrent.futures import ThreadPoolExecutor
        self.compact = bool(compact)
        self.nw = max(1, int(streams))
        self.patch, self.exact = patch_size, exact_f64
        self.device = torch.cuda.current_device()
        self.streams = [torch.cuda.Stream() for _ in range(self.nw)]
        self.stages = [HostStage() for _ in range(self.nw)]
        self.up = [None] * self.nw
        self.pool = ThreadPoolExecutor(self.nw)
        self.last_d2h_bytes = 0
        device_tables(torch.device("cuda", self.device))

    def _work(self, w, grids, download):
        torch.cuda.set_device(self.device)
        out = []
        with torch.cuda.stream(self.streams[w]):
            for j in range(w, len(grids), self.nw):
                g = grids[j]
                if isinstance(g, np.ndarray):
                    g = torch.from_numpy(np.ascontiguousarray(g, dtype=np.float32))
                if not g.is_cuda:
                    if self.up[w] is None or self.up[w].shape != g.shape:
                        self.up[w] = torch.empty(tuple(g.shape), dtype=torch.float32, device="cuda")
                    self.up[w].copy_(g, non_blocking=True)
                    g = self.up[w]
                sp, kp, ori, dsc = describe_struct(g, patch_size=self.patch, exact_f64=self.exact)
                r = {"n_kp": len(kp), "n_dsc": len(ori)}
                if download:
                    st = self.stages[w]
                    r.update(kp=st.fetch("kp%d" % j, kp.table[:len(kp)]), ori=st.fetch("ori%d" % j, ori.table[:len(ori)]))
                    if self.compact:
                        ds = DescriptorSet(dsc)
                        r["_max"] = ds._max_dev[:1]
                        r["dsc_u8"] = st.fetch("dsc8_%d" % j, ds.u8[:ds.rows])
                        r["_dsc_dev"] = dsc
                    else:
                        r["dsc"] = st.fetch("dsc%d" % j, dsc)
                else:
                    r.update(dsc=dsc, kp=kp.table[:len(kp)], ori=ori.table[:len(ori)])
                out.append((j, r))
            self.streams[w].synchronize()
            for _, r in out:
                if "_max" in r:
                    if int(r.pop("_max").item()) > 255:
                        del r["dsc_u8"]
                        r["dsc"] = r["_dsc_dev"].cpu()
                    del r["_dsc_dev"]
        return out

    def run(self, grids, download=True):
        main = torch.cuda.current_stream()
        for s_ in self.streams:
            s_.wait_stream(main)
        parts = [f.result() for f in [self.pool.submit(self._work, w, grids, download) for w in range(self.nw)]]
        for s_ in self.streams:
            main.wait_stream(s_)
        res = [r for _, r in sorted((x for p in parts for x in p), key=lambda x: x[0])]
        if download:
            self.last_d2h_bytes = int(sum(r[k].numel() * r[k].element_size() for r in res for k in ("dsc", "dsc_u8", "kp", "ori") if k in r))
        return res


def concat_sets(sets):
    offs = np.cumsum([0] + [s.rows for s in sets]).astype(np.int64)
    return DescriptorSet(torch.cat([s.dsc for s in sets], 0)), offs


def match_topk(hi, lo, k=8, lo_index_base=0, impl=None):
    hi, lo = _as_set(hi), _as_set(lo)
    dev = hi.dsc.device
    st = _stream()
    impl, verify = _pick_impl(hi, lo, impl)
    idx = torch.empty((hi.rows, k), dtype=torch.int32, device=dev)
    score = torch.empty((hi.rows, k), dtype=torch.float64, device=dev)
    ws_bytes = _lib.lib.mad_match_topk_workspace_bytes(hi.rows, lo.rows, int(k), impl)
    ws = torch.empty(ws_bytes, dtype=torch.uint8, device=dev)
    call("mad_match_topk", C.byref(hi.c), C.byref(lo.c), int(k), int(lo_index_base), _ptr(idx), _ptr(score), _ptr(ws),
         ws_bytes, impl, st)
    if verify:
        _read_counts(torch.zeros(1, dtype=torch.int64, device=dev), hi, lo)
        if _exact_impl(hi, lo) != 0:
            return match_topk(hi, lo, k, lo_index_base)
    return idx, score


def topk_merge(idx_g, score_g):
    g, m, k = idx_g.shape
    dev = idx_g.device
    idx = torch.empty((m, k), dtype=torch.int32, device=dev)
    score = torch.empty((m, k), dtype=torch.float64, device=dev)
    call("mad_topk_merge", _ptr(idx_g.contiguous()), _ptr(score_g.contiguous()), g, m, k, _ptr(idx), _ptr(score), _stream())
    return idx, score


class FeatureTable(object):

    def __init__(self, dsc, index, oct_scale, main_bin, sec_bin, subv_map_coords):
        _require_cuda()
        self.set = dsc if isinstance(dsc, DescriptorSet) else DescriptorSet(dsc)
        dev = self.set.dsc.device
        meta = np.stack([np.asarray(index), np.asarray(oct_scale), np.asarray(main_bin), np.asarray(sec_bin)], 1)
        self.meta_host = np.ascontiguousarray(meta, dtype=np.int32)
        self.subv_host = np.ascontiguousarray(subv_map_coords, dtype=np.float64).reshape(-1, 3)
        assert len(self.meta_host) == self.set.rows == len(self.subv_host)
        self.meta = torch.from_numpy(self.meta_host).to(dev)
        self.subv = torch.from_numpy(self.subv_host).to(dev)

    @classmethod
    def from_features(cls, df_list):
        dsc = np.array([df.lin_ar_subeqsp for df in df_list], dtype=np.int16).reshape(-1, DSC_LEN)
        return cls(dsc, [df.index for df in df_list], [df.oct_scale for df in df_list], [df.main_bin for df in df_list],
                   [df.sec_bin for df in df_list], np.array([df.subv_map_coords for df in df_list], dtype=np.float64))


class AnchorCloud(object):

    def __init__(self, subv, used, cell):
        dev = subv.device
        st = _stream()
        d = int(subv.shape[0])
        self.cell = float(cell)
        self._buf = torch.empty((max(d, 1), 3), dtype=torch.float64, device=dev)
        self.org_dev = torch.empty(3, dtype=torch.float64, device=dev)
        self.info = torch.empty(8, dtype=torch.int64, device=dev)
        ws_bytes = _lib.lib.mad_anchor_cloud_workspace_bytes(d)
        ws = torch.empty(ws_bytes, dtype=torch.uint8, device=dev)
        call("mad_anchor_cloud", _ptr(subv), _ptr(used), d, C.c_double(self.cell), _ptr(self._buf), _ptr(self.org_dev),
             _ptr(self.info), _ptr(ws), ws_bytes, st)
        self.n = None

    def take_info(self, vals):
        n, bad = int(vals[0]), int(vals[1])
        if bad:
            raise _lib.MadError("anchor cloud: %d used feature(s) with a non-finite coordinate" % bad)
        self.n = n
        self.dims64 = np.array(vals[2:5], dtype=np.int64)
        self.org = np.array(vals[5:8], dtype=np.int64).view(np.float64)
        self.dims = self.dims64.astype(np.int32)
        self.cloud = self._buf[:n]
        return self

    def build_grid(self):
        dev = self._buf.device
        ncell = int(np.prod([int(v) for v in self.dims64], dtype=object))
        fits = ncell < (1 << 31)
        self.sorted = torch.empty((max(self.n, 1), 3), dtype=torch.float64, device=dev)
        self.cell_start = torch.empty(ncell + 1 if fits else 1, dtype=torch.int32, device=dev)
        self.near_bits = torch.zeros((ncell + 31) // 32 if fits else 1, dtype=torch.int32, device=dev)
        ws_bytes = _lib.lib.mad_cloud_grid_workspace_bytes(self.n)
        ws = torch.empty(ws_bytes, dtype=torch.uint8, device=dev)
        call("mad_cloud_grid", _ptr(self.cloud), self.n, _ptr(self.org_dev), _dptr(self.dims64), C.c_double(self.cell),
             _ptr(self.sorted), _ptr(self.cell_start) if fits else None, _ptr(self.near_bits) if fits else None, _ptr(ws),
             ws_bytes, _stream())
        self.sorted = self.sorted[:self.n]
        return self

    def host(self):
        return self.cloud.cpu().numpy()


def read_clouds(*clouds):
    vals = _Readback.read(*[c.info for c in clouds])
    return [c.take_info(vals[8 * i:8 * i + 8]) for i, c in enumerate(clouds)]


def anchor_cloud(subv, used, cell):
    c, = read_clouds(AnchorCloud(subv.contiguous(), used.contiguous(), cell))
    return c.build_grid()


class DscMatch(object):

    def __init__(self, lo, hi, anchor_dist_thresh=4, cc_threshold=0.65, impl=None, pairs=None):
        self.lo, self.hi = lo, hi
        self.dist = float(anchor_dist_thresh)
        dev = hi.set.dsc.device
        if pairs is None:
            pairs = match_threshold(hi.set, lo.set, cc_threshold, impl=impl)
        self.ph, self.pl, self.sc = pairs
        self.p = int(self.ph.numel())
        self.hi_cloud = self.lo_cloud = None
        if self.p == 0:
            return
        st = _stream()
        used_hi = torch.zeros(hi.set.rows, dtype=torch.uint8, device=dev)
        used_lo = torch.zeros(lo.set.rows, dtype=torch.uint8, device=dev)
        call("mad_mark_used", _ptr(self.ph), self.p, _ptr(used_hi), st)
        call("mad_mark_used", _ptr(self.pl), self.p, _ptr(used_lo), st)
        self.hi_cloud, self.lo_cloud = read_clouds(AnchorCloud(hi.subv, used_hi, self.dist),
                                                   AnchorCloud(lo.subv, used_lo, self.dist))
        self.lo_cloud.build_grid()
        self.tb = device_tables(dev)

    def _common(self):
        return (_ptr(self.hi.subv), _ptr(self.lo.subv), _ptr(self.hi.meta), _ptr(self.lo.meta), _ptr(self.tb.rf),
                _ptr(self.tb.rf_inv), self.tb.ori_zones)

    def _grid(self):
        g = self.lo_cloud
        return (_ptr(self.hi_cloud.cloud), self.hi_cloud.n, _ptr(g.sorted), _ptr(g.cell_start), _ptr(g.near_bits), _dptr(g.org),
                _dptr(g.dims), C.c_double(self.dist))

    def counts(self, p0, p1):
        out = torch.empty(max(p1 - p0, 1), dtype=torch.int32, device=self.ph.device)
        if p1 > p0:
            call("mad_repeat_counts", _ptr(self.ph), _ptr(self.pl), int(p0), int(p1), *self._common(), *self._grid(), _ptr(out),
                 _stream())
        return out[:p1 - p0]

    def rows(self, counts):
        if counts.numel() != self.p or counts.dtype != torch.int32 or counts.device != self.ph.device:
            raise _lib.MadError("DscMatch.rows: needs int32 counts of all %d pairs on %s, got %s [%d] on %s"
                                % (self.p, self.ph.device, counts.dtype, counts.numel(), counts.device))
        res = torch.empty((self.p, 23), dtype=torch.float64, device=self.ph.device)
        call("mad_repeat_rows", _ptr(self.ph), _ptr(self.pl), _ptr(self.sc), self.p, *self._common(), _ptr(counts.contiguous()),
             self.hi_cloud.n, _ptr(res), _stream())
        return res

    def table(self):
        res = torch.empty((self.p, 23), dtype=torch.float64, device=self.ph.device)
        call("mad_repeatability", _ptr(self.ph), _ptr(self.pl), _ptr(self.sc), self.p, *self._common(), *self._grid(), _ptr(res),
             _stream())
        return res

    def result(self, table):
        if self.p == 0:
            return table, np.zeros((0, 3)), np.zeros((0, 3))
        return table, self.lo_cloud.host(), self.hi_cloud.host()

    def empty(self):
        return torch.empty((0, 23), dtype=torch.float64, device=self.ph.device)


def match_dsc(lo, hi, anchor_dist_thresh=4, cc_threshold=0.65, impl=None):
    m = DscMatch(lo, hi, anchor_dist_thresh, cc_threshold, impl)
    return m.result(m.table() if m.p else m.empty())


def match_dsc_lists(lo_dsc_list, hi_dsc_list, anchor_dist_thresh=4, cc_threshold=0.65):
    res, lo_cloud, hi_cloud = match_dsc(FeatureTable.from_features(lo_dsc_list), FeatureTable.from_features(hi_dsc_list),
                                        anchor_dist_thresh, cc_threshold)
    return list(res.cpu().numpy()), lo_cloud, hi_cloud
```

Before: 2.243 billion.

## Process keypoints in spatial order and batch all orientation rotations in one pass

Adds a keypoint ordering kernel so orient and describe blocks visit keypoints in spatial order, improving cache locality of gradient reads, and carries a feature order through compaction into describe. The orient kernel is restructured: the patch gradients are stored as SoA floats, histograms for all main orientations are accumulated in a single pass over the patch instead of one pass per main zone, and secondary selection uses warp ballots. It also adds launch bounds for occupancy. This costs more shared memory for the extra histograms and an extra single-block ordering launch.

```diff
diff --git a/include/mad_b200.h b/include/mad_b200.h
--- a/include/mad_b200.h
+++ b/include/mad_b200.h
@@ -98,15 +98,31 @@
                const double* r1_table, int lim_main, int lim_sec,
                int32_t* n_ori, int32_t* slots, void* stream);
 
+int mad_keypoint_order(const MadKeypoint* kp, int n_kp, int32_t* kp_order, void* stream);
+
+int mad_orient_ordered(const float* grad4_oct0, const float* grad4_oct1, const int* dims_oct_host,
+                       const MadKeypoint* kp, const int32_t* kp_order, int n_kp, int r,
+                       const MadZoneTable* zones112_host, const double* r1_table, int lim_main, int lim_sec,
+                       int32_t* n_ori, int32_t* slots, void* stream);
+
 size_t mad_compact_oriented_workspace_bytes(int n_kp);
 int mad_compact_oriented(const int32_t* n_ori, const int32_t* slots, int n_kp,
                          MadOriented* oriented, int cap, int* out_count,
                          void* workspace, size_t workspace_bytes, void* stream);
 
+int mad_compact_oriented_ordered(const int32_t* n_ori, const int32_t* slots, const int32_t* kp_order, int n_kp,
+                                 MadOriented* oriented, int cap, int* out_count, int32_t* feat_order,
+                                 void* workspace, size_t workspace_bytes, void* stream);
+
 int mad_describe(const float* grad4_oct0, const float* grad4_oct1, const int* dims_oct_host,
                  const MadKeypoint* kp, const MadOriented* oriented, int n_oriented, int r,
                  const MadZoneTable* zones16_host, const double* rf_table, const double* rf_inv_table,
                  int rf_zones, int16_t* dsc, void* stream);
+
+int mad_describe_ordered(const float* grad4_oct0, const float* grad4_oct1, const int* dims_oct_host,
+                         const MadKeypoint* kp, const MadOriented* oriented, const int32_t* feat_order,
+                         int n_oriented, int r, const MadZoneTable* zones16_host, const double* rf_table,
+                         const double* rf_inv_table, int rf_zones, int16_t* dsc, void* stream);
 
 typedef struct MadDscSet {
     const int16_t* dsc;
diff --git a/mad_b200/_lib.py b/mad_b200/_lib.py
--- a/mad_b200/_lib.py
+++ b/mad_b200/_lib.py
@@ -77,7 +77,11 @@
     "mad_orient": (_I, [_P, _P, _P, _P, _I, _I, C.POINTER(MadZoneTable), _P, _I, _I, _P, _P, _P]),
     "mad_compact_oriented_workspace_bytes": (_SZ, [_I]),
     "mad_compact_oriented": (_I, [_P, _P, _I, _P, _I, _P, _P, _SZ, _P]),
+    "mad_keypoint_order": (_I, [_P, _I, _P, _P]),
+    "mad_orient_ordered": (_I, [_P, _P, _P, _P, _P, _I, _I, C.POINTER(MadZoneTable), _P, _I, _I, _P, _P, _P]),
+    "mad_compact_oriented_ordered": (_I, [_P, _P, _P, _I, _P, _I, _P, _P, _P, _SZ, _P]),
     "mad_describe": (_I, [_P, _P, _P, _P, _P, _I, _I, C.POINTER(MadZoneTable), _P, _P, _I, _P, _P]),
+    "mad_describe_ordered": (_I, [_P, _P, _P, _P, _P, _P, _I, _I, C.POINTER(MadZoneTable), _P, _P, _I, _P, _P]),
     "mad_dsc_prepare": (_I, [_P, _I, _I, _P, _P, _P, _P, _P, _P]),
     "mad_match_pairs": (_I, [C.POINTER(MadDscSet), C.POINTER(MadDscSet), C.c_double, _P, _P, C.c_uint64, _P, _P]),
     "mad_match_pairs_finish_workspace_bytes": (_SZ, [C.c_longlong]),
diff --git a/mad_b200/csrc/describe.cu b/mad_b200/csrc/describe.cu
--- a/mad_b200/csrc/describe.cu
+++ b/mad_b200/csrc/describe.cu
@@ -23,18 +23,19 @@
     return 0;
 }
 
-template <int NB, int SIDE, int THREADS>
+template <int NB, int SIDE, int THREADS, bool ORDERED>
 __global__ void __launch_bounds__(THREADS, 768 / THREADS)
 describe_kernel(const float4* __restrict__ grad0, const float4* __restrict__ grad1, OctDims dims,
-                const MadKeypoint* __restrict__ kp, const MadOriented* __restrict__ oriented, int r,
-                ZoneTab T, const double* __restrict__ rf_table, const double* __restrict__ rf_inv_table,
+                const MadKeypoint* __restrict__ kp, const MadOriented* __restrict__ oriented,
+                const int32_t* __restrict__ feat_order, int r, ZoneTab T, const double* __restrict__ rf_table, const double* __restrict__ rf_inv_table,
                 int rf_zones, int16_t* __restrict__ dsc) {
     __shared__ int cnt[MAD_DSC_LEN];
     __shared__ ZoneFast F;
     __shared__ double xt[32][3];
     const int tid = threadIdx.x;
     if (SIDE) r = SIDE / 2;
-    const MadOriented of = oriented[blockIdx.x];
+    const int f = ORDERED ? feat_order[blockIdx.x] : blockIdx.x;
+    const MadOriented of = oriented[f];
     const MadKeypoint K = kp[of.kp];
     const int o = K.oct ? 1 : 0;
     const float4* __restrict__ grad = o ? grad1 : grad0;
@@ -70,8 +71,8 @@
     const int s_bad = __syncthreads_or(bad);
     float vz_hi[NB];
     zone_fast_hi<NB>(F, vz_hi);
-    int16_t* out = dsc + (long long)blockIdx.x * MAD_DSC_LEN;
     if (s_bad) {
+        int16_t* out = dsc + (long long)f * MAD_DSC_LEN;
         for (int q = tid; q < MAD_DSC_LEN; q += blockDim.x) out[q] = 0;
         return;
     }
@@ -129,15 +130,16 @@
         }
     }
     __syncthreads();
+    int16_t* out = dsc + (long long)(ORDERED ? feat_order[blockIdx.x] : blockIdx.x) * MAD_DSC_LEN;
     for (int q = tid; q < MAD_DSC_LEN; q += blockDim.x) out[q] = (int16_t)cnt[q];
 }
 
 }
 
-extern "C" int mad_describe(const float* grad4_oct0, const float* grad4_oct1, const int* dims_oct_host,
-                            const MadKeypoint* kp, const MadOriented* oriented, int n_oriented, int r,
-                            const MadZoneTable* zones_host, const double* rf_table, const double* rf_inv_table,
-                            int rf_zones, int16_t* dsc, void* stream) {
+extern "C" int mad_describe_ordered(const float* grad4_oct0, const float* grad4_oct1, const int* dims_oct_host,
+                                    const MadKeypoint* kp, const MadOriented* oriented, const int32_t* feat_order,
+                                    int n_oriented, int r, const MadZoneTable* zones_host, const double* rf_table,
+                                    const double* rf_inv_table, int rf_zones, int16_t* dsc, void* stream) {
     MAD_CHECK_ARG(dims_oct_host && zones_host && n_oriented >= 0);
     if (n_oriented == 0) return MAD_OK;
     MAD_CHECK_ARG(grad4_oct0 && grad4_oct1 && kp && oriented && rf_table && rf_inv_table && dsc);
@@ -154,12 +156,27 @@
         MAD_CHECK_ARG((long long)d.n[o][0] * d.n[o][1] * d.n[o][2] < (1LL << 31));
     auto launch = [&](auto kernel, int threads) {
         kernel<<<n_oriented, threads, 0, (cudaStream_t)stream>>>(
-            reinterpret_cast<const float4*>(grad4_oct0), reinterpret_cast<const float4*>(grad4_oct1), d, kp, oriented, r,
-            T, rf_table, rf_inv_table, rf_zones, dsc);
+            reinterpret_cast<const float4*>(grad4_oct0), reinterpret_cast<const float4*>(grad4_oct1), d, kp, oriented,
+            feat_order, r, T, rf_table, rf_inv_table, rf_zones, dsc);
     };
-    if (T.n_belts <= 4 && r == 8) launch(describe_kernel<4, 16, 128>, 128);
-    else if (T.n_belts <= 4) launch(describe_kernel<4, 0, 256>, 256);
-    else launch(describe_kernel<MAD_BELT_MAX, 0, 256>, 256);
+    if (T.n_belts <= 4 && r == 8) {
+        if (feat_order) launch(describe_kernel<4, 16, 128, true>, 128);
+        else launch(describe_kernel<4, 16, 128, false>, 128);
+    } else if (T.n_belts <= 4) {
+        if (feat_order) launch(describe_kernel<4, 0, 256, true>, 256);
+        else launch(describe_kernel<4, 0, 256, false>, 256);
+    } else {
+        if (feat_order) launch(describe_kernel<MAD_BELT_MAX, 0, 256, true>, 256);
+        else launch(describe_kernel<MAD_BELT_MAX, 0, 256, false>, 256);
+    }
     MAD_LAUNCH_OK();
     return MAD_OK;
 }
+
+extern "C" int mad_describe(const float* grad4_oct0, const float* grad4_oct1, const int* dims_oct_host,
+                            const MadKeypoint* kp, const MadOriented* oriented, int n_oriented, int r,
+                            const MadZoneTable* zones_host, const double* rf_table, const double* rf_inv_table,
+                            int rf_zones, int16_t* dsc, void* stream) {
+    return mad_describe_ordered(grad4_oct0, grad4_oct1, dims_oct_host, kp, oriented, nullptr, n_oriented, r, zones_host,
+                                rf_table, rf_inv_table, rf_zones, dsc, stream);
+}
diff --git a/mad_b200/csrc/orient.cu b/mad_b200/csrc/orient.cu
--- a/mad_b200/csrc/orient.cu
+++ b/mad_b200/csrc/orient.cu
@@ -63,22 +63,63 @@
     return total;
 }
 
+#define MAD_ORI_THREADS 128
+#define MAD_ORI_MAIN_MAX 6
+
+__device__ __forceinline__ int secondaries_warp(const int* h, int n_zones, int lim_sec, int* sec) {
+    const int lane = threadIdx.x & 31;
+    int hv[4], hm = 0;
+#pragma unroll
+    for (int k = 0; k < 4; ++k) {
+        const int z = lane + 32 * k;
+        hv[k] = (z < n_zones) ? h[z] : 0;
+        hm = max(hm, hv[k]);
+    }
+#pragma unroll
+    for (int d = 16; d > 0; d >>= 1) hm = max(hm, __shfl_xor_sync(0xFFFFFFFFu, hm, d));
+    if (hm == 0) return 0;
+    int cur[4], qmax = 0;
+#pragma unroll
+    for (int k = 0; k < 4; ++k) {
+        const int z = lane + 32 * k;
+        cur[k] = norm50(hv[k], hm);
+        if (z >= 1 && z < n_zones - 1) qmax = max(qmax, cur[k]);
+    }
+#pragma unroll
+    for (int d = 16; d > 0; d >>= 1) qmax = max(qmax, __shfl_xor_sync(0xFFFFFFFFu, qmax, d));
+    if (qmax == 0) return 0;
+    int ns = 0;
+#pragma unroll
+    for (int k = 0; k < 4; ++k) {
+        const int z = lane + 32 * k;
+        const bool f = z >= 1 && z < n_zones - 1 && norm50(cur[k], qmax) > 40;
+        const unsigned m = __ballot_sync(0xFFFFFFFFu, f);
+        const int p = ns + __popc(m & ((1u << lane) - 1u));
+        if (f && p < 8) sec[p] = z;
+        ns += __popc(m);
+    }
+    return ns <= lim_sec ? ns : 0;
+}
+
 template <int NB>
-__global__ void __launch_bounds__(128)
+__global__ void __launch_bounds__(MAD_ORI_THREADS, 7)
 orient_kernel(const float4* __restrict__ grad0, const float4* __restrict__ grad1, OctDims dims,
-              const MadKeypoint* __restrict__ kp, int r, const char4* __restrict__ mask_off, int n_mask,
-              ZoneTab T, const double* __restrict__ r1_table, int lim_main, int lim_sec,
-              int32_t* __restrict__ n_ori, int32_t* __restrict__ slots) {
-    extern __shared__ float4 pv[];
-    __shared__ int hist[128];
-    __shared__ int hn0[128];
-    __shared__ int cur[128];
-    __shared__ int s_main[8], s_sec[8], s_wcnt[8];
-    __shared__ int s_hmax, s_count;
+              const MadKeypoint* __restrict__ kp, const int32_t* __restrict__ order, int r,
+              const char4* __restrict__ mask_off, int n_mask, ZoneTab T, const double* __restrict__ r1_table,
+              int lim_main, int lim_sec, int32_t* __restrict__ n_ori, int32_t* __restrict__ slots) {
+    extern __shared__ float pv[];
+    __shared__ int hist[1 + MAD_ORI_MAIN_MAX][128];
+    __shared__ int s_main[8], s_wcnt[8];
+    __shared__ int s_sec[MAD_ORI_MAIN_MAX][8], s_npair[MAD_ORI_MAIN_MAX];
+    __shared__ float s_rf[MAD_ORI_MAIN_MAX][9];
+    __shared__ int s_hmax;
     __shared__ ZoneFast F;
+    float* const px = pv;
+    float* const py = pv + n_mask;
+    float* const pz = pv + 2 * n_mask;
 
     const int tid = threadIdx.x;
-    const int ki = blockIdx.x;
+    const int ki = order ? order[blockIdx.x] : blockIdx.x;
     const MadKeypoint K = kp[ki];
     const int o = K.oct ? 1 : 0;
     const float4* __restrict__ grad = o ? grad1 : grad0;
@@ -90,19 +131,19 @@
         if (tid == 0) n_ori[ki] = 0;
         return;
     }
-    if (tid < 128) { hist[tid] = 0; }
-    if (tid == 0) { s_hmax = 0; s_count = 0; }
+    for (int q = tid; q < (1 + MAD_ORI_MAIN_MAX) * 128; q += MAD_ORI_THREADS) (&hist[0][0])[q] = 0;
+    if (tid == 0) s_hmax = 0;
     zone_fast_init(&F, T);
     __syncthreads();
     float vz_hi[NB];
     zone_fast_hi<NB>(F, vz_hi);
 
     constexpr int GB = 4;
-    for (int i0 = tid; i0 < n_mask; i0 += GB * blockDim.x) {
+    for (int i0 = tid; i0 < n_mask; i0 += GB * MAD_ORI_THREADS) {
         float4 gv[GB];
 #pragma unroll
         for (int u = 0; u < GB; ++u) {
-            const int i = i0 + u * blockDim.x;
+            const int i = i0 + u * MAD_ORI_THREADS;
             gv[u] = make_float4(0.f, 0.f, 0.f, 0.f);
             if (i < n_mask) {
                 const char4 d = mask_off[i];
@@ -122,97 +163,91 @@
         }
 #pragma unroll
         for (int u = 0; u < GB; ++u) {
-            const int i = i0 + u * blockDim.x;
+            const int i = i0 + u * MAD_ORI_THREADS;
             if (i < n_mask) {
-                pv[i] = gv[u];
+                px[i] = gv[u].x; py[i] = gv[u].y; pz[i] = gv[u].z;
                 if (gv[u].w != 0.f) {
-                    if (zf[u] >= 0) atomicAdd(&hist[zf[u]], 1);
-                    else vote_exact_f32(T, gv[u].x, gv[u].y, gv[u].z, hist);
+                    if (zf[u] >= 0) atomicAdd(&hist[0][zf[u]], 1);
+                    else vote_exact_f32(T, gv[u].x, gv[u].y, gv[u].z, hist[0]);
                 }
             }
         }
     }
     __syncthreads();
-    if (tid < T.n_zones) atomicMax(&s_hmax, hist[tid]);
+    if (tid < T.n_zones) atomicMax(&s_hmax, hist[0][tid]);
     __syncthreads();
     const int hmax0 = s_hmax;
     if (hmax0 == 0) {
         if (tid == 0) n_ori[ki] = 0;
         return;
     }
-    if (tid < T.n_zones) hn0[tid] = norm50(hist[tid], hmax0);
-    __syncthreads();
-    const int nmain = select_zones(tid < T.n_zones && hn0[tid] > 40, tid, s_main, s_wcnt);
+    const int nmain = select_zones(tid < T.n_zones && norm50(hist[0][tid], hmax0) > 40, tid, s_main, s_wcnt);
     if (nmain > lim_main) {
         if (tid == 0) n_ori[ki] = 0;
         return;
     }
 
-    for (int mi = 0; mi < nmain; ++mi) {
-        const int a = s_main[mi];
-        bool have = true;
-        if (a != 0) {
-            if (tid < 128) hist[tid] = 0;
-            if (tid == 0) s_hmax = 0;
-            __syncthreads();
-            const double* R = r1_table + 9 * a;
+    const int first = s_main[0] != 0 ? 1 : 0;
+    const int nrot = nmain - 1 + first;
+    if (tid < 9 * nrot) s_rf[tid / 9][tid % 9] = (float)r1_table[9 * s_main[tid / 9 + 1 - first] + tid % 9];
+    __syncthreads();
+    for (int i0 = tid; i0 < n_mask; i0 += GB * MAD_ORI_THREADS) {
+        float gx[GB], gy[GB], gz[GB], gw[GB];
+#pragma unroll
+        for (int u = 0; u < GB; ++u) {
+            const int i = min(i0 + u * MAD_ORI_THREADS, n_mask - 1);
+            gx[u] = px[i]; gy[u] = py[i]; gz[u] = pz[i];
+            const float m2 = __fadd_rn(__fadd_rn(__fmul_rn(gx[u], gx[u]), __fmul_rn(gy[u], gy[u])), __fmul_rn(gz[u], gz[u]));
+            const float rinv = mad_rsqrt_approx(fmaxf(m2, 1e-30f));
+            gw[u] = (i0 + u * MAD_ORI_THREADS >= n_mask || m2 < MAD_M2_LT) ? 0.f : ((m2 >= MAD_M2_GT) ? rinv : -1.f);
+        }
+#pragma unroll 1
+        for (int c = 0; c < nrot; ++c) {
             float rf[9];
 #pragma unroll
-            for (int q = 0; q < 9; ++q) rf[q] = (float)R[q];
-            for (int i0 = tid; i0 < n_mask; i0 += GB * blockDim.x) {
-                float4 gq[GB];
-                int zq[GB];
-#pragma unroll
-                for (int u = 0; u < GB; ++u) {
-                    const int i = min(i0 + u * (int)blockDim.x, n_mask - 1);
-                    const float4 g = pv[i];
-                    gq[u] = g;
-                    const float vx = fmaf(g.z, rf[2], fmaf(g.y, rf[1], g.x * rf[0])) * g.w;
-                    const float vy = fmaf(g.z, rf[5], fmaf(g.y, rf[4], g.x * rf[3])) * g.w;
-                    const float vz = fmaf(g.z, rf[8], fmaf(g.y, rf[7], g.x * rf[6])) * g.w;
-                    zq[u] = (g.w > 0.f) ? zone_fast<NB>(F, vz_hi, vx, vy, vz) : -1;
-                }
-#pragma unroll
-                for (int u = 0; u < GB; ++u) {
-                    if (i0 + u * (int)blockDim.x < n_mask && gq[u].w != 0.f) {
-                        if (zq[u] >= 0) atomicAdd(&hist[zq[u]], 1);
-                        else vote_exact_f64(T, R, gq[u].x, gq[u].y, gq[u].z, hist);
-                    }
+            for (int q = 0; q < 9; ++q) rf[q] = s_rf[c][q];
+            int zq[GB];
+#pragma unroll
+            for (int u = 0; u < GB; ++u) {
+                const float vx = fmaf(gz[u], rf[2], fmaf(gy[u], rf[1], gx[u] * rf[0])) * gw[u];
+                const float vy = fmaf(gz[u], rf[5], fmaf(gy[u], rf[4], gx[u] * rf[3])) * gw[u];
+                const float vz = fmaf(gz[u], rf[8], fmaf(gy[u], rf[7], gx[u] * rf[6])) * gw[u];
+                zq[u] = (gw[u] > 0.f) ? zone_fast<NB>(F, vz_hi, vx, vy, vz) : -1;
+            }
+#pragma unroll
+            for (int u = 0; u < GB; ++u) {
+                if (gw[u] != 0.f) {
+                    if (zq[u] >= 0) atomicAdd(&hist[1 + c][zq[u]], 1);
+                    else vote_exact_f64(T, r1_table + 9 * s_main[c + 1 - first], gx[u], gy[u], gz[u], hist[1 + c]);
                 }
             }
-            __syncthreads();
-            if (tid < T.n_zones) atomicMax(&s_hmax, hist[tid]);
-            __syncthreads();
-            const int hm = s_hmax;
-            if (hm == 0) have = false;
-            else if (tid < T.n_zones) cur[tid] = norm50(hist[tid], hm);
-        } else {
-            if (tid < T.n_zones) cur[tid] = hn0[tid];
-        }
-        __syncthreads();
-        if (tid == 0) s_hmax = 0;
-        __syncthreads();
-        const bool inner = tid >= 1 && tid < T.n_zones - 1;
-        if (have && inner) atomicMax(&s_hmax, cur[tid]);
-        __syncthreads();
-        const int qmax = s_hmax;
-        const int ns = select_zones(have && inner && qmax > 0 && norm50(cur[tid], max(qmax, 1)) > 40, tid, s_sec, s_wcnt);
-        if (tid == 0 && have && qmax > 0 && ns <= lim_sec) {
-            int c = s_count;
-            for (int q = 0; q < ns && c < MAD_MAX_ORI; ++q) slots[(long long)ki * MAD_MAX_ORI + c++] = a | (s_sec[q] << 16);
-            s_count = c;
-        }
-        __syncthreads();
-    }
-    if (tid == 0) n_ori[ki] = s_count;
+        }
+    }
+    __syncthreads();
+
+    const int warp = tid >> 5;
+    for (int mi = warp; mi < nmain; mi += MAD_ORI_THREADS / 32) {
+        const int np = secondaries_warp(hist[mi + first], T.n_zones, lim_sec, s_sec[mi]);
+        if ((tid & 31) == 0) s_npair[mi] = np;
+    }
+    __syncthreads();
+    int base = 0;
+    for (int mi = 0; mi < nmain; ++mi) {
+        const int q = tid - base;
+        if (q >= 0 && q < s_npair[mi] && tid < MAD_MAX_ORI)
+            slots[(long long)ki * MAD_MAX_ORI + tid] = s_main[mi] | (s_sec[mi][q] << 16);
+        base += s_npair[mi];
+    }
+    if (tid == 0) n_ori[ki] = min(base, MAD_MAX_ORI);
 }
 
 __global__ void compact_oriented_kernel(const int32_t* __restrict__ n_ori, const int32_t* __restrict__ slots,
-                                        const int* __restrict__ pos, int n_kp, MadOriented* __restrict__ out,
-                                        int cap, int* __restrict__ out_count) {
-    const int i = blockIdx.x * blockDim.x + threadIdx.x;
-    if (i >= n_kp) return;
-    const int n = n_ori[i], p = pos[i];
+                                        const int* __restrict__ pos, const int32_t* __restrict__ order, int n_kp,
+                                        MadOriented* __restrict__ out, int cap, int* __restrict__ out_count,
+                                        int32_t* __restrict__ feat_order, int* __restrict__ feat_count) {
+    const int b = blockIdx.x * blockDim.x + threadIdx.x;
+    const int i = b < n_kp ? (order ? order[b] : b) : -1;
+    const int n = i >= 0 ? n_ori[i] : 0, p = i >= 0 ? pos[i] : 0;
     for (int q = 0; q < n; ++q) {
         if (p + q < cap) {
             const int v = slots[(long long)i * MAD_MAX_ORI + q];
@@ -224,6 +259,75 @@
         }
     }
     if (i == n_kp - 1) *out_count = p + n;
+    if (order) {
+        const int lane = threadIdx.x & 31;
+        int incl = n;
+#pragma unroll
+        for (int d = 1; d < 32; d <<= 1) {
+            const int t = __shfl_up_sync(0xFFFFFFFFu, incl, d);
+            if (lane >= d) incl += t;
+        }
+        const int total = __shfl_sync(0xFFFFFFFFu, incl, 31);
+        int base = 0;
+        if (lane == 31 && total > 0) base = atomicAdd(feat_count, total);
+        base = __shfl_sync(0xFFFFFFFFu, base, 31) + incl - n;
+        for (int q = 0; q < n; ++q) feat_order[base + q] = p + q;
+    }
+}
+
+#define MAD_ORDER_BUCKETS 8192
+#define MAD_ORDER_THREADS 1024
+__device__ __forceinline__ uint32_t spread3_4(uint32_t v) {
+    v &= 0xFu;
+    v = (v | (v << 4)) & 0x0C3u;
+    v = (v | (v << 2)) & 0x249u;
+    return v;
+}
+__device__ __forceinline__ int spatial_bucket(const MadKeypoint& K) {
+    const int o = K.oct ? 1 : 0;
+    const int sh = 5 - o;
+    return (o << 12) | (int)((spread3_4((uint32_t)K.vox[0] >> sh) << 2) | (spread3_4((uint32_t)K.vox[1] >> sh) << 1) |
+                             spread3_4((uint32_t)K.vox[2] >> sh));
+}
+
+__global__ void __launch_bounds__(MAD_ORDER_THREADS)
+keypoint_order_kernel(const MadKeypoint* __restrict__ kp, int n_kp, int32_t* __restrict__ order) {
+    using Scan = cub::BlockScan<int, MAD_ORDER_THREADS>;
+    constexpr int PER = MAD_ORDER_BUCKETS / MAD_ORDER_THREADS;
+    __shared__ int cnt[MAD_ORDER_BUCKETS];
+    __shared__ typename Scan::TempStorage tmp;
+    for (int q = threadIdx.x; q < MAD_ORDER_BUCKETS; q += MAD_ORDER_THREADS) cnt[q] = 0;
+    __syncthreads();
+    constexpr int GB = 8;
+    for (int i0 = threadIdx.x; i0 < n_kp; i0 += GB * MAD_ORDER_THREADS) {
+        int bk[GB];
+#pragma unroll
+        for (int u = 0; u < GB; ++u) {
+            const int i = i0 + u * MAD_ORDER_THREADS;
+            bk[u] = i < n_kp ? spatial_bucket(kp[i]) : -1;
+        }
+#pragma unroll
+        for (int u = 0; u < GB; ++u) if (bk[u] >= 0) atomicAdd(&cnt[bk[u]], 1);
+    }
+    __syncthreads();
+    int c[PER], sum = 0;
+#pragma unroll
+    for (int u = 0; u < PER; ++u) { c[u] = cnt[threadIdx.x * PER + u]; sum += c[u]; }
+    int base;
+    Scan(tmp).ExclusiveSum(sum, base);
+#pragma unroll
+    for (int u = 0; u < PER; ++u) { cnt[threadIdx.x * PER + u] = base; base += c[u]; }
+    __syncthreads();
+    for (int i0 = threadIdx.x; i0 < n_kp; i0 += GB * MAD_ORDER_THREADS) {
+        int bk[GB];
+#pragma unroll
+        for (int u = 0; u < GB; ++u) {
+            const int i = i0 + u * MAD_ORDER_THREADS;
+            bk[u] = i < n_kp ? spatial_bucket(kp[i]) : -1;
+        }
+#pragma unroll
+        for (int u = 0; u < GB; ++u) if (bk[u] >= 0) order[atomicAdd(&cnt[bk[u]], 1)] = i0 + u * MAD_ORDER_THREADS;
+    }
 }
 
 }
@@ -257,10 +361,10 @@
     return MAD_OK;
 }
 
-extern "C" int mad_orient(const float* grad4_oct0, const float* grad4_oct1, const int* dims_oct_host,
-                          const MadKeypoint* kp, int n_kp, int r, const MadZoneTable* zones_host,
-                          const double* r1_table, int lim_main, int lim_sec, int32_t* n_ori, int32_t* slots,
-                          void* stream) {
+extern "C" int mad_orient_ordered(const float* grad4_oct0, const float* grad4_oct1, const int* dims_oct_host,
+                                  const MadKeypoint* kp, const int32_t* kp_order, int n_kp, int r,
+                                  const MadZoneTable* zones_host, const double* r1_table, int lim_main, int lim_sec,
+                                  int32_t* n_ori, int32_t* slots, void* stream) {
     MAD_CHECK_ARG(dims_oct_host && zones_host && r1_table && n_kp >= 0);
     if (n_kp == 0) return MAD_OK;
     MAD_CHECK_ARG(grad4_oct0 && grad4_oct1 && kp && n_ori && slots);
@@ -275,16 +379,15 @@
     ZoneTab T;
     T.bounds = zones_host->bounds; T.belt_first = zones_host->belt_first; T.belt_phi = zones_host->belt_phi;
     T.n_zones = zones_host->n_zones; T.n_belts = zones_host->n_belts; T.fast = zones_host->fast;
-    const size_t smem = (size_t)n_mask * sizeof(float4);
+    const size_t smem = (size_t)n_mask * 3 * sizeof(float);
     if (smem > 200 * 1024) { mad_set_error("mad_orient: patch radius %d too large", r); return MAD_ERR_ARG; }
     MAD_CHECK_ARG(T.n_belts >= 1 && T.n_belts <= MAD_BELT_MAX && T.n_zones <= MAD_ZONE_MAX);
     auto launch = [&](auto kernel) -> int {
         MAD_CUDA(cudaFuncSetAttribute(kernel, cudaFuncAttributeMaxDynamicSharedMemorySize, (int)std::max<size_t>(smem, 48 * 1024)));
         MAD_PROF("orient_kernel", stream);
-        kernel<<<n_kp, 128, smem, (cudaStream_t)stream>>>(
-
-            reinterpret_cast<const float4*>(grad4_oct0), reinterpret_cast<const float4*>(grad4_oct1), d, kp, r, mask,
-            n_mask, T, r1_table, lim_main, lim_sec, n_ori, slots);
+        kernel<<<n_kp, MAD_ORI_THREADS, smem, (cudaStream_t)stream>>>(
+            reinterpret_cast<const float4*>(grad4_oct0), reinterpret_cast<const float4*>(grad4_oct1), d, kp, kp_order, r,
+            mask, n_mask, T, r1_table, lim_main, lim_sec, n_ori, slots);
         return MAD_OK;
     };
     int lrc;
@@ -294,6 +397,14 @@
     if (lrc != MAD_OK) return lrc;
     MAD_LAUNCH_OK();
     return MAD_OK;
+}
+
+extern "C" int mad_orient(const float* grad4_oct0, const float* grad4_oct1, const int* dims_oct_host,
+                          const MadKeypoint* kp, int n_kp, int r, const MadZoneTable* zones_host,
+                          const double* r1_table, int lim_main, int lim_sec, int32_t* n_ori, int32_t* slots,
+                          void* stream) {
+    return mad_orient_ordered(grad4_oct0, grad4_oct1, dims_oct_host, kp, nullptr, n_kp, r, zones_host, r1_table,
+                              lim_main, lim_sec, n_ori, slots, stream);
 }
 
 __global__ void zone_fast_build_kernel(ZoneTab T, ZoneFast* out) {
@@ -319,14 +430,27 @@
     return MAD_OK;
 }
 
+extern "C" int mad_keypoint_order(const MadKeypoint* kp, int n_kp, int32_t* kp_order, void* stream) {
+    MAD_CHECK_ARG(n_kp >= 0);
+    if (n_kp == 0) return MAD_OK;
+    MAD_CHECK_ARG(kp && kp_order);
+    MAD_PROF("keypoint_order_kernel", stream);
+    keypoint_order_kernel<<<1, MAD_ORDER_THREADS, 0, (cudaStream_t)stream>>>(kp, n_kp, kp_order);
+    MAD_LAUNCH_OK();
+    return MAD_OK;
+}
+
 extern "C" size_t mad_compact_oriented_workspace_bytes(int n_kp) {
     size_t b = 0;
-    cub::DeviceScan::ExclusiveSum(nullptr, b, (const int*)nullptr, (int*)nullptr, n_kp > 0 ? n_kp : 1);
-    return mad_align_up((size_t)(n_kp > 0 ? n_kp : 1) * sizeof(int), 256) + mad_align_up(b, 256);
-}
-
-extern "C" int mad_compact_oriented(const int32_t* n_ori, const int32_t* slots, int n_kp, MadOriented* oriented,
-                                    int cap, int* out_count, void* workspace, size_t workspace_bytes, void* stream) {
+    const int n = n_kp > 0 ? n_kp : 1;
+    cub::DeviceScan::ExclusiveSum(nullptr, b, (const int*)nullptr, (int*)nullptr, n);
+    return mad_align_up((size_t)n * sizeof(int), 256) + 256 + mad_align_up(b, 256);
+}
+
+extern "C" int mad_compact_oriented_ordered(const int32_t* n_ori, const int32_t* slots, const int32_t* kp_order,
+                                            int n_kp, MadOriented* oriented, int cap, int* out_count,
+                                            int32_t* feat_order, void* workspace, size_t workspace_bytes,
+                                            void* stream) {
     MAD_CHECK_ARG(out_count && n_kp >= 0);
     cudaStream_t st = (cudaStream_t)stream;
     if (n_kp == 0) {
@@ -335,15 +459,26 @@
     }
     MAD_CHECK_ARG(n_ori && slots && oriented && workspace && cap >= 0);
     MAD_CHECK_ARG(workspace_bytes >= mad_compact_oriented_workspace_bytes(n_kp));
+    MAD_CHECK_ARG(!kp_order || (feat_order && (long long)cap >= (long long)n_kp * MAD_MAX_ORI));
+    const size_t arr = mad_align_up((size_t)n_kp * sizeof(int), 256);
     int* pos = reinterpret_cast<int*>(workspace);
-    char* cub_ws = reinterpret_cast<char*>(workspace) + mad_align_up((size_t)n_kp * sizeof(int), 256);
-    size_t cub_bytes = workspace_bytes - mad_align_up((size_t)n_kp * sizeof(int), 256);
+    int* feat_count = reinterpret_cast<int*>(reinterpret_cast<char*>(workspace) + arr);
+    char* cub_ws = reinterpret_cast<char*>(workspace) + arr + 256;
+    size_t cub_bytes = workspace_bytes - arr - 256;
+    if (kp_order) MAD_CUDA(cudaMemsetAsync(feat_count, 0, sizeof(int), st));
     {
         MAD_PROF("cub_exclusive_sum", st);
         MAD_CUDA(cub::DeviceScan::ExclusiveSum(cub_ws, cub_bytes, n_ori, pos, n_kp, st));
     }
     MAD_PROF("compact_oriented_kernel", st);
-    compact_oriented_kernel<<<(int)mad_ceil_div(n_kp, 256), 256, 0, st>>>(n_ori, slots, pos, n_kp, oriented, cap, out_count);
+    compact_oriented_kernel<<<(int)mad_ceil_div(n_kp, 256), 256, 0, st>>>(n_ori, slots, pos, kp_order, n_kp, oriented,
+                                                                          cap, out_count, feat_order, feat_count);
     MAD_LAUNCH_OK();
     return MAD_OK;
 }
+
+extern "C" int mad_compact_oriented(const int32_t* n_ori, const int32_t* slots, int n_kp, MadOriented* oriented,
+                                    int cap, int* out_count, void* workspace, size_t workspace_bytes, void* stream) {
+    return mad_compact_oriented_ordered(n_ori, slots, nullptr, n_kp, oriented, cap, out_count, nullptr, workspace,
+                                        workspace_bytes, stream);
+}
diff --git a/mad_b200/pipeline.py b/mad_b200/pipeline.py
--- a/mad_b200/pipeline.py
+++ b/mad_b200/pipeline.py
@@ -290,9 +290,10 @@
 
 
 class Oriented(object):
-    def __init__(self, table, count):
+    def __init__(self, table, count, feat_order=None):
         self.table = table
         self.count = int(count)
+        self.feat_order = feat_order
         self._host = None
 
     def host(self):
@@ -312,7 +313,14 @@
     return o
 
 
-def orient(space, kp, radius=8, lim_main=6, lim_sec=6):
+def keypoint_order(kp):
+    n = len(kp)
+    order = torch.empty(max(n, 1), dtype=torch.int32, device=kp.table.device)
+    call("mad_keypoint_order", _ptr(kp.table), n, _ptr(order), _stream())
+    return order
+
+
+def orient(space, kp, radius=8, lim_main=6, lim_sec=6, spatial_order=True):
     _require_cuda()
     dev = space.grad4[0].device
     st = _stream()
@@ -321,18 +329,21 @@
     if n == 0:
         return Oriented(torch.empty((1, 2), dtype=torch.int32, device=dev), 0)
     ensure_gradient(space, kp, radius)
+    order = keypoint_order(kp) if spatial_order else None
     n_ori = torch.empty(n, dtype=torch.int32, device=dev)
     slots = torch.empty((n, MAX_ORI), dtype=torch.int32, device=dev)
     dims = space.dims_host
-    call("mad_orient", _ptr(space.grad4[0]), _ptr(space.grad4[1]), _dptr(dims), _ptr(kp.table), n, int(radius),
-         C.byref(tb.z_ori), _ptr(tb.r1), int(lim_main), int(lim_sec), _ptr(n_ori), _ptr(slots), st)
+    call("mad_orient_ordered", _ptr(space.grad4[0]), _ptr(space.grad4[1]), _dptr(dims), _ptr(kp.table), _ptr(order),
+         n, int(radius), C.byref(tb.z_ori), _ptr(tb.r1), int(lim_main), int(lim_sec), _ptr(n_ori), _ptr(slots), st)
     cap = n * MAX_ORI
     out = torch.empty((cap, 2), dtype=torch.int32, device=dev)
     out_count = torch.zeros(1, dtype=torch.int32, device=dev)
+    feat_order = torch.empty(cap, dtype=torch.int32, device=dev) if spatial_order else None
     ws_bytes = _lib.lib.mad_compact_oriented_workspace_bytes(n)
     ws = torch.empty(ws_bytes, dtype=torch.uint8, device=dev)
-    call("mad_compact_oriented", _ptr(n_ori), _ptr(slots), n, _ptr(out), cap, _ptr(out_count), _ptr(ws), ws_bytes, st)
-    return Oriented(out, _Readback.read(out_count)[0])
+    call("mad_compact_oriented_ordered", _ptr(n_ori), _ptr(slots), _ptr(order), n, _ptr(out), cap, _ptr(out_count),
+         _ptr(feat_order), _ptr(ws), ws_bytes, st)
+    return Oriented(out, _Readback.read(out_count)[0], feat_order)
 
 
 def describe(space, kp, ori, radius=8):
@@ -346,8 +357,9 @@
         return dsc
     ensure_gradient(space, kp, radius)
     dims = space.dims_host
-    call("mad_describe", _ptr(space.grad4[0]), _ptr(space.grad4[1]), _dptr(dims), _ptr(kp.table), _ptr(ori.table), d,
-         int(radius), C.byref(tb.z_dsc), _ptr(tb.rf), _ptr(tb.rf_inv), tb.ori_zones, _ptr(dsc), st)
+    call("mad_describe_ordered", _ptr(space.grad4[0]), _ptr(space.grad4[1]), _dptr(dims), _ptr(kp.table),
+         _ptr(ori.table), _ptr(ori.feat_order), d, int(radius), C.byref(tb.z_dsc), _ptr(tb.rf), _ptr(tb.rf_inv),
+         tb.ori_zones, _ptr(dsc), st)
     return dsc
 
 
```

Measured after the change: 2.250 billion (median of 6 runs). Within noise of the previous version (+0.3%).
